# Guoxs/DODT

Measured on AMD Instinct MI355X. Metric: frame-pairs/sec (whole node) KITTI-shape tau=2, higher is better.
Workload: dtype f32

## Files before the change

dodt_amd/_lib.py:

```python
import ctypes as C
import os

_HERE = os.path.dirname(os.path.abspath(__file__))
LIB_PATH = os.environ.get('DODT_HIP_LIB') or os.path.join(_HERE, 'lib', 'libdodt_hip.so')

OK, ERR_INVALID, ERR_HIP, ERR_UNSUPPORTED = 0, 1, 2, 3
PTS_VELO_XYZI, PTS_CAM_3XN = 0, 1
EXTRACTOR_VGG_PYR = 0
EXTRACTOR_VGG = 1
EXTRACTOR_SHARED_GPU = 0x100
EXTRACTOR_BF16 = 0x200
EXTRACTOR_SPLIT = 0x400
FC_RELU = 1
FC_BF16 = 2
CONFLICT_RAISE, CONFLICT_NEXT_BEST = 0, 1


class DodtError(RuntimeError):
    pass


class BevParams(C.Structure):
    _fields_ = [
        ('point_format', C.c_int32),
        ('num_slices', C.c_int32),
        ('velo_to_cam', C.c_double * 12),
        ('p2', C.c_double * 12),
        ('im_w', C.c_double),
        ('im_h', C.c_double),
        ('plane', C.c_double * 4),
        ('extents', C.c_double * 6),
        ('voxel_size', C.c_double),
        ('height_lo', C.c_double),
        ('height_hi', C.c_double),
        ('occ_lo', C.c_double),
        ('occ_hi', C.c_double),
        ('has_pre_transform', C.c_int32),
        ('reserved_', C.c_int32),
        ('pre_translate', C.c_double * 3),
        ('pre_rotate', C.c_double * 9),
    ]


class LayerInfo(C.Structure):
    _fields_ = [('name', C.c_char * 32), ('kernel', C.c_char * 48), ('launches', C.c_int32),
                ('items', C.c_int32), ('flops_direct', C.c_double), ('flops_executed', C.c_double),
                ('bytes', C.c_double), ('ms', C.c_float), ('reserved_', C.c_int32)]


_vp = C.c_void_p
_i = C.c_int
_f = C.c_float
_d = C.c_double
_pi32 = C.c_void_p
_pf = C.c_void_p
_hf = C.c_void_p

SIGNATURES = {
    'dodt_version': (_i, []),
    'dodt_last_error': (C.c_char_p, []),
    'dodt_ctx_create': (_i, [_i, C.POINTER(_vp)]),
    'dodt_mark': (_i, [_vp, _i]),
    'dodt_ctx_wait_mark': (_i, [_vp, _vp, _i]),
    'dodt_mark_elapsed': (_i, [_vp, _i, _vp, _i, C.POINTER(_f)]),
    'dodt_ctx_create_high_priority': (_i, [_i, C.POINTER(_vp)]),
    'dodt_ctx_create_on_stream': (_i, [_i, _vp, C.POINTER(_vp)]),
    'dodt_ctx_destroy': (_i, [_vp]),
    'dodt_ctx_sync': (_i, [_vp]),
    'dodt_ctx_wait_for': (_i, [_vp, _vp]),
    'dodt_malloc': (_i, [_vp, C.c_size_t, C.POINTER(_vp)]),
    'dodt_free': (_i, [_vp, _vp]),
    'dodt_memcpy_h2d': (_i, [_vp, _vp, _vp, C.c_size_t]),
    'dodt_memcpy_d2h': (_i, [_vp, _vp, _vp, C.c_size_t]),
    'dodt_memset': (_i, [_vp, _vp, _i, C.c_size_t]),
    'dodt_pinned_alloc': (_i, [_vp, C.c_size_t, C.POINTER(_vp)]),
    'dodt_pinned_free': (_i, [_vp, _vp]),
    'dodt_memcpy_h2d_async': (_i, [_vp, _vp, _vp, C.c_size_t]),
    'dodt_fetch_i32_begin': (_i, [_vp, _pi32, _i, _i]),
    'dodt_fetch_i32_end': (_i, [_vp, _i, C.POINTER(C.c_int32), _i]),
    'dodt_timer_start': (_i, [_vp]),
    'dodt_timer_stop': (_i, [_vp, C.POINTER(_f)]),
    'dodt_bev_slices': (_i, [_vp, _vp, _i, C.POINTER(BevParams), _pf, _vp]),
    'dodt_bev_status': (_i, [_vp, C.POINTER(_i)]),
    'dodt_bev_support_mask': (_i, [C.POINTER(BevParams), _i, _vp, _i, _i]),
    'dodt_anchor_filter': (_i, [_vp, _vp, _i, _i, _pi32, _i, _i, _pi32, _pi32]),
    'dodt_project_anchors_f64': (_i, [_vp, _vp, _pi32, _i, _pi32,
                                      C.POINTER(_d), C.POINTER(_d), _d, _d,
                                      _pf, _pf, _pf]),
    'dodt_project_anchors_f32': (_i, [_vp, _pf, _i, _pi32, C.POINTER(_f),
                                      C.POINTER(_f), _f, _f, _pf, _pf, _pf]),
    'dodt_img_preprocess': (_i, [_vp, _vp, _i, _i, _i, _i, _i,
                                 C.POINTER(_f), _pf]),
    'dodt_conv_mode': (_i, []),
    'dodt_extractor_create': (_i, [_vp, _i, _i, _i, _i, _i, _i,
                                   C.POINTER(_vp)]),
    'dodt_extractor_destroy': (_i, [_vp]),
    'dodt_extractor_set_layer': (_i, [_vp, C.c_char_p, _vp, _i, _i, _i, _i,
                                      _vp, _vp, _vp]),
    'dodt_extractor_input': (_i, [_vp, C.POINTER(_vp), C.POINTER(C.c_longlong)]),
    'dodt_extractor_forward': (_i, [_vp, _pf, _pf, _pf]),
    'dodt_extractor_forward_padded': (_i, [_vp, _pf, _pf, _pf]),
    'dodt_extractor_set_input': (_i, [_vp, _pf]),
    'dodt_extractor_set_input_support': (_i, [_vp, _vp, _i, _i, C.POINTER(C.c_longlong)]),
    'dodt_extractor_set_frame_tables': (_i, [_vp, _i, C.POINTER(_i)]),
    'dodt_extractor_frame_items': (_i, [_vp, C.POINTER(_i), _i]),
    'dodt_extractor_frame_split': (_i, [_vp, C.POINTER(_i), C.POINTER(_i), _i]),
    'dodt_extractor_store_bytes': (C.c_longlong, [_vp]),
    'dodt_frame_tables_host': (_i, [_vp, _i, _i, _i, _i, _i, _i, _vp, _i, _vp, _vp, C.POINTER(_i)]),
    'dodt_frame_restore_host': (_i, [_vp, _i, _i, _i, _i, _i, _i, _i, _i, _i, _vp, _vp, _vp, _vp]),
    'dodt_frame_lists_host': (_i, [_vp, _i, _i, _i, _i, _i, _i, _vp, _i, _vp, _vp, C.POINTER(_i), _vp, C.POINTER(_i)]),
    'dodt_extractor_read_activation': (_i, [_vp, C.c_char_p, _vp,
                                            C.POINTER(_i), C.POINTER(_i),
                                            C.POINTER(_i)]),
    'dodt_extractor_output_shape': (_i, [_vp, C.POINTER(_i), C.POINTER(_i), C.POINTER(_i)]),
    'dodt_extractor_first_layers_folded': (_i, [_vp]),
    'dodt_extractor_flops': (_d, [_vp]),
    'dodt_extractor_mfma_flops': (_d, [_vp]),
    'dodt_extractor_bytes': (_d, [_vp]),
    'dodt_extractor_layer_count': (_i, [_vp]),
    'dodt_extractor_forward_timed': (_i, [_vp, _pf, _pf, _pf, C.POINTER(LayerInfo), _i]),
    'dodt_crop_and_resize': (_i, [_vp, _pf, _i, _i, _i, _pf, _i, _pi32, _i, _i,
                                  _pf]),
    'dodt_crop_and_resize_strided': (_i, [_vp, _pf, _i, _i, _i, _pf, _i, _pi32, _i, _i, _pf,
                                          C.c_longlong]),
    'dodt_correlation': (_i, [_vp, _pf, _pf, _i, _i, _i, _i, _i, _i, _pf]),
    'dodt_crop_and_resize_indexed': (_i, [_vp, _pf, _i, _i, _i, _pf, _i, _pi32, _i, _pi32, _i, _i, _pf,
                                          C.c_longlong]),
    'dodt_correlation_tile_list': (_i, [_vp, _i, _i, _pf, _i, _pi32, _i, _pi32, _i, _i, _pi32, _i, _pi32]),
    'dodt_correlation_tiles': (_i, [_vp, _pf, _pf, _i, _i, _i, _i, _i, _i, _pi32, _i, _pi32, _pf]),
    'dodt_mean_fusion': (_i, [_vp, _pf, _pf, _i, _pi32, _i, _pf]),
    'dodt_fc_create': (_i, [_vp, _i, _i, _hf, _hf, _i, C.POINTER(_vp)]),
    'dodt_fc_create_ex': (_i, [_vp, _i, _i, _hf, _hf, _i, C.POINTER(_vp)]),
    'dodt_fc_destroy': (_i, [_vp]),
    'dodt_fc_forward': (_i, [_vp, _vp, _pf, _pf, _i, _i, _pi32, _pf, _i]),
    'dodt_fc_forward_split': (_i, [_vp, _vp, _pf, _i, _i, _pi32, _i, C.POINTER(_i), C.POINTER(_vp)]),
    'dodt_fc_flops': (_d, [_vp, _i]),
    'dodt_fc_bf16_row_elems': (_i, [_vp]),
    'dodt_fc_forward_bf16': (_i, [_vp, _vp, _vp, _i, _i, _pi32, _vp, _i, _i]),
    'dodt_fc_forward_split_bf16': (_i, [_vp, _vp, _vp, _i, _i, _pi32, _i, C.POINTER(_i), C.POINTER(_vp)]),
    'dodt_rows_to_bf16': (_i, [_vp, _pf, _pf, _i, _pi32, _i, _i, _vp, _i]),
    'dodt_nms': (_i, [_vp, _pf, _pf, _i, _pi32, _i, _f, _pi32, _pi32]),
    'dodt_offset_to_anchor': (_i, [_vp, _pf, _pf, _i, _pi32, _pf]),
    'dodt_softmax_fg': (_i, [_vp, _pf, _i, _pi32, _pf]),
    'dodt_rpn_decode': (_i, [_vp, _pf, _pf, _pf, _i, _pi32, C.POINTER(_f), _pf, _pf, _pf]),
    'dodt_gather_project': (_i, [_vp, _pf, _pi32, _i, _pi32, C.POINTER(_f), C.POINTER(_f), _f, _f, _pf, _pf, _pf]),
    'dodt_final_decode': (_i, [_vp, _pf, _pf, _pf, _pf, _i, _pi32, C.POINTER(_f), C.POINTER(_f),
                               _pf, _pf, _pf, _pf, _pf, _pf]),
    'dodt_gather_rows': (_i, [_vp, _pf, _i, _pi32, _i, _pi32, _pf]),
    'dodt_max_fg_logit': (_i, [_vp, _pf, _i, _i, _pi32, _pf]),
    'dodt_pack_detections': (_i, [_vp, _pf, _pf, _pf, _pf, _pi32, _pi32, _i, _f, _pf, _pi32]),
    'dodt_pack_detections_compact': (_i, [_vp, _pf, _pf, _pf, _pf, _pi32, _pi32, _i, _f, _pf, _pi32]),
    'dodt_angle_vector_to_orientation': (_i, [_vp, _pf, _i, _pi32, _pf]),
    'dodt_class_scores': (_i, [_vp, _pf, _i, _i, _pi32, _pf, _pi32]),
    'dodt_final_decode_classes': (_i, [_vp, _pf, _pf, _pf, _i, _pf, _i, _pi32, C.POINTER(_f), C.POINTER(_f),
                                       _pf, _pf, _pf, _pf, _pf, _pi32, _pf]),
    'dodt_pack_detections_classes': (_i, [_vp, _pf, _pf, _pi32, _pf, _pf, _pi32, _pi32, _i, _f, _pf, _pi32]),
    'dodt_pack_detections_compact_classes': (_i, [_vp, _pf, _pf, _pi32, _pf, _pf, _pi32, _pi32, _i, _f, _pf, _pi32]),
    'dodt_box_4c_decode': (_i, [_vp, _pf, _pf, _i, _pi32, C.POINTER(_f),
                                C.POINTER(_f), _pf, _pf, _pf]),
    'dodt_comm_unique_id': (_i, [_vp]),
    'dodt_comm_create': (_i, [_vp, _i, _i, _vp, C.POINTER(_vp)]),
    'dodt_comm_destroy': (_i, [_vp]),
    'dodt_comm_attach': (_i, [_vp, _vp]),
    'dodt_comm_rank': (_i, [_vp, C.POINTER(_i), C.POINTER(_i)]),
    'dodt_comm_set_late_peer': (_i, [_vp, _d]),
    'dodt_all_gather_records': (_i, [_vp, _vp, _i, _pf, _pi32, _i, _i, _i, _i, _pf, _pi32]),
    'dodt_comm_join': (_i, [_vp, _i, _vp]),
    'dodt_comm_sync': (_i, [_vp]),
    'dodt_comm_barrier': (_i, [_vp]),
    'dodt_comm_max_f64': (_i, [_vp, C.POINTER(_d)]),
    'dodt_three_d_iou_matrix': (_i, [_vp, _vp, _i, _vp, _i, _vp]),
    'dodt_interpolate_pairs': (_i, [_vp, _vp, _i, _pi32, _i, _i, _i, _d, _i, _vp, C.POINTER(_d), _i, _vp,
                                    _pi32, _pi32]),
    'dodt_track_state_bytes': (_i, [_i, C.POINTER(C.c_size_t)]),
    'dodt_track_reset': (_i, [_vp, _vp, _i]),
    'dodt_track_flush': (_i, [_vp, _vp, _d, _i]),
    'dodt_track_encode': (_i, [_vp, _vp, _i, _pi32, _i, _i, C.POINTER(_d), _d, _d, _d, _pf, _pf, _pi32]),
    'dodt_track_pairs': (_i, [_vp, _vp, _vp, _i, _pi32, _i, _i, C.POINTER(_d), _d, _d, _d, _d, _d, _i]),
    'dodt_track_encoded': (_i, [_vp, _vp, _pf, _pf, _pi32, _i, _i, _d, _d, _i]),
}
COMM_ID_BYTES = 128

_lib = None


def load():
    global _lib
    if _lib is not None:
        return _lib
    if not os.path.exists(LIB_PATH):
        raise DodtError(
            'libdodt_hip.so not found at %s -- build it with '
            '`make -C dodt_amd/csrc` (there is no CPU fallback)' % LIB_PATH)
    lib = C.CDLL(LIB_PATH)
    for name, (res, args) in SIGNATURES.items():
        fn = getattr(lib, name)
        fn.restype = res
        fn.argtypes = args
    _lib = lib
    return lib


def check(rc, what=''):
    if rc == OK:
        return
    msg = load().dodt_last_error().decode('utf-8', 'replace')
    if rc == ERR_INVALID:
        raise ValueError(msg or what)
    raise DodtError('%s: %s (status %d)' % (what, msg, rc))
```

dodt_amd/core/models/anchor_predictor.py:

```python
import numpy as np

from dodt_amd import ops


class AnchorPredictor(object):
    def __init__(self, ctx, params, dtype='f32'):
        def mat(name):
            w = np.asarray(params[name]['w'], np.float32)
            return w.reshape(-1, w.shape[-1]), np.asarray(params[name]['b'], np.float32)
        wc, bc = mat('cls_fc6')
        wr, br = mat('reg_fc6')
        self.width = wc.shape[1]
        if wr.shape != wc.shape:
            raise ValueError('cls_fc6 and reg_fc6 must have the same size')
        self.fc6 = ops.FullyConnected(ctx, np.concatenate([wc, wr], 1),
                                      np.concatenate([bc, br]), True, dtype=dtype)
        self.cls7 = ops.FullyConnected(ctx, *mat('cls_fc7'), relu=True, dtype=dtype)
        self.reg7 = ops.FullyConnected(ctx, *mat('reg_fc7'), relu=True, dtype=dtype)
        self.cls8 = ops.FullyConnected(ctx, *mat('cls_fc8'), relu=False, dtype=dtype)
        self.reg8 = ops.FullyConnected(ctx, *mat('reg_fc8'), relu=False, dtype=dtype)
        self.layers = [self.fc6, self.cls7, self.reg7, self.cls8, self.reg8]
        (w8c, b8c), (w8r, b8r) = mat('cls_fc8'), mat('reg_fc8')
        w8 = np.zeros((w8c.shape[0] + w8r.shape[0], w8c.shape[1] + w8r.shape[1]), np.float32)
        w8[:w8c.shape[0], :w8c.shape[1]] = w8c
        w8[w8c.shape[0]:, w8c.shape[1]:] = w8r
        self.out8 = ops.FullyConnected(ctx, w8, np.concatenate([b8c, b8r]), False, dtype=dtype)
        if not (self.out8.can_split() and w8c.shape[0] == self.width == w8r.shape[0]):
            self.out8.close()
            self.out8 = None
        self.ctx = ctx

    def make_scratch(self, n_max):
        return [self.ctx.empty((n_max, 2 * self.width), np.float32) for _ in range(2)]

    def forward(self, ctx, d_bev_roi, d_img_roi, n, d_objectness, d_offsets, scratch):
        w = self.width
        h6, h7 = scratch
        self.fc6.forward(d_bev_roi, n, h6, d_x2=d_img_roi, ctx=ctx)
        self.cls7.forward(h6, n, h7, ldx=2 * w, ldy=2 * w, ctx=ctx)
        self.reg7.forward(h6.offset(4 * w, (1,)), n, h7.offset(4 * w, (1,)),
                          ldx=2 * w, ldy=2 * w, ctx=ctx)
        if self.out8 is not None:
            self.out8.forward_split(h7, n, [d_objectness, d_offsets], [self.cls8.N, self.reg8.N], ctx=ctx)
            return
        self.cls8.forward(h7, n, d_objectness, ldx=2 * w, ctx=ctx)
        self.reg8.forward(h7.offset(4 * w, (1,)), n, d_offsets, ldx=2 * w, ctx=ctx)

    def flops(self, n):
        return sum(l.flops(n) for l in self.layers)

    def close(self):
        for l in self.layers + ([self.out8] if self.out8 is not None else []):
            l.close()
```

dodt_amd/csrc/anchors.hip:

```cpp
#include "common.h"

namespace {

__device__ __forceinline__ int box_count(const uint32_t* __restrict__ occ, int wpr, int x1,
                                         int z1, int x2, int z2, int thr) {
    int cnt = 0;
    if (x2 <= x1) return 0;
    const int w0 = x1 >> 5, w1 = (x2 - 1) >> 5;
    for (int z = z1; z < z2; ++z) {
        for (int w = w0; w <= w1; ++w) {
            uint32_t word = occ[z * wpr + w];
            const int lo = (w == w0) ? (x1 & 31) : 0;
            const int hi = (w == w1) ? ((x2 - 1) & 31) : 31;
            uint32_t m = (hi == 31 ? 0xFFFFFFFFu : ((1u << (hi + 1)) - 1u)) & ~((1u << lo) - 1u);
            cnt += __popc(word & m);
        }
        if (cnt >= thr) return cnt;
    }
    return cnt;
}

constexpr int kMaskBlock = 64;
__global__ void __launch_bounds__(kMaskBlock)
anchor_mask_kernel(const uint32_t* __restrict__ occ, int wpr, int nx, int nz,
                   const int4* __restrict__ cells, int n, int thr,
                   uint8_t* __restrict__ mask, int* __restrict__ block_counts) {
    const int i = blockIdx.x * blockDim.x + threadIdx.x;
    int keep = 0;
    if (i < n) {
        int4 b = cells[i];
        const int x1 = min(max(b.x, 0), nx), z1 = min(max(b.y, 0), nz);
        const int x2 = min(max(b.z, 0), nx), z2 = min(max(b.w, 0), nz);
        keep = box_count(occ, wpr, x1, z1, x2, z2, thr) >= thr;
        mask[i] = (uint8_t)keep;
    }
    const int total = __popcll(__ballot(keep));
    if (threadIdx.x == 0) block_counts[blockIdx.x] = total;
}

__global__ void __launch_bounds__(256)
anchor_compact_kernel(const uint8_t* __restrict__ mask, const int* __restrict__ block_counts,
                      int n, int* __restrict__ keep_idx, int* __restrict__ count_out) {
    __shared__ int s_part[256];
    __shared__ int s_wave[4];
    const int tid = threadIdx.x;
    int part = 0;
    for (int j = tid; j < (int)blockIdx.x * (256 / kMaskBlock); j += 256) part += block_counts[j];
    s_part[tid] = part;
    __syncthreads();
    for (int s = 128; s > 0; s >>= 1) {
        if (tid < s) s_part[tid] += s_part[tid + s];
        __syncthreads();
    }
    const int block_off = s_part[0];
    const int i = blockIdx.x * 256 + tid;
    const int keep = (i < n) ? mask[i] : 0;
    const unsigned long long bal = __ballot(keep);
    const int lane = tid & 63, wave = tid >> 6;
    const int before = __popcll(bal & ((1ull << lane) - 1ull));
    if (lane == 0) s_wave[wave] = __popcll(bal);
    __syncthreads();
    int wave_off = 0;
    for (int w = 0; w < wave; ++w) wave_off += s_wave[w];
    if (keep) keep_idx[block_off + wave_off + before] = i;
    if (blockIdx.x == gridDim.x - 1 && tid == 0)
        *count_out = block_off + s_wave[0] + s_wave[1] + s_wave[2] + s_wave[3];
}

struct ProjParams64 {
    double x_min, x_max, z_min, z_max;
    double p[12];
    double im_w, im_h;
};

__device__ __forceinline__ void proj_corner64(const double* p, double x, double y, double z,
                                              double& u, double& v) {
    const double un = fma(p[2], z, fma(p[1], y, p[0] * x)) + p[3];
    const double vn = fma(p[6], z, fma(p[5], y, p[4] * x)) + p[7];
    const double w = fma(p[10], z, fma(p[9], y, p[8] * x)) + p[11];
    u = un / w;
    v = vn / w;
}

__global__ void __launch_bounds__(256)
project_f64_kernel(const double* __restrict__ anchors, const int* __restrict__ idx, int n,
                   const int* __restrict__ d_n, const ProjParams64 P,
                   float* __restrict__ bev_norm, float* __restrict__ img_norm,
                   float* __restrict__ anchors_f32) {
    const int i = blockIdx.x * blockDim.x + threadIdx.x;
    const int lim = d_n ? min(*d_n, n) : n;
    if (i >= lim) return;
    const int row = idx ? idx[i] : i;
    const double* a = anchors + (size_t)row * 6;
    const double x = a[0], y = a[1], z = a[2], dx = a[3], dy = a[4], dz = a[5];
    if (anchors_f32) {
        float* o = anchors_f32 + (size_t)i * 6;
        o[0] = (float)x; o[1] = (float)y; o[2] = (float)z;
        o[3] = (float)dx; o[4] = (float)dy; o[5] = (float)dz;
    }
    const double hx = dx / 2.0, hz = dz / 2.0;
    if (bev_norm) {
        const double xr = P.x_max - P.x_min, zr = P.z_max - P.z_min;
        const double x1 = (x - hx) - P.x_min, x2 = (x + hx) - P.x_min;
        const double z1 = (P.z_max - (z + hz)) - P.z_min, z2 = (P.z_max - (z - hz)) - P.z_min;
        float* o = bev_norm + (size_t)i * 4;
        o[0] = (float)(z1 / zr); o[1] = (float)(x1 / xr);
        o[2] = (float)(z2 / zr); o[3] = (float)(x2 / xr);
    }
    if (img_norm) {
        double umin = 1e300, umax = -1e300, vmin = 1e300, vmax = -1e300;
        const double xs[2] = {x + hx, x - hx};
        const double ys[2] = {y, y - dy};
        const double zs[2] = {z + hz, z - hz};
#pragma unroll
        for (int k = 0; k < 8; ++k) {
            double u, v;
            proj_corner64(P.p, xs[(k >> 1) & 1], ys[k >> 2], zs[((k + 1) >> 1) & 1], u, v);
            umin = (u < umin || u != u) ? u : umin; umax = (u > umax || u != u) ? u : umax;
            vmin = (v < vmin || v != v) ? v : vmin; vmax = (v > vmax || v != v) ? v : vmax;
        }
        float* o = img_norm + (size_t)i * 4;
        o[0] = (float)(vmin / P.im_h); o[1] = (float)(umin / P.im_w);
        o[2] = (float)(vmax / P.im_h); o[3] = (float)(umax / P.im_w);
    }
}

struct ProjParams32 {
    float x_min, x_max, z_min, z_max;
    float p[12];
    float im_w, im_h;
};

__device__ __forceinline__ void bev_box32(float x, float z, float dx, float dz,
                                          const ProjParams32& P, float& x1, float& z1,
                                          float& x2, float& z2) {
    const float hx = dx / 2.0f, hz = dz / 2.0f;
    x1 = (x - hx) - P.x_min;
    x2 = (x + hx) - P.x_min;
    z1 = (P.z_max - (z + hz)) - P.z_min;
    z2 = (P.z_max - (z - hz)) - P.z_min;
}

__device__ __forceinline__ void project_f32_elem(int i, float x, float y, float z, float dx, float dy, float dz,
                                                 const ProjParams32& P, float* __restrict__ bev,
                                                 float* __restrict__ bev_norm_tf, float* __restrict__ img_norm_tf) {
    float x1, z1, x2, z2;
    bev_box32(x, z, dx, dz, P, x1, z1, x2, z2);
    if (bev) {
        float* o = bev + (size_t)i * 4;
        o[0] = x1; o[1] = z1; o[2] = x2; o[3] = z2;
    }
    if (bev_norm_tf) {
        const float xr = P.x_max - P.x_min, zr = P.z_max - P.z_min;
        float* o = bev_norm_tf + (size_t)i * 4;
        o[0] = z1 / zr; o[1] = x1 / xr; o[2] = z2 / zr; o[3] = x2 / xr;
    }
    if (img_norm_tf) {
        const float hx = dx / 2.0f, hz = dz / 2.0f;
        const float xs[2] = {x + hx, x - hx};
        const float ys[2] = {y, y - dy};
        const float zs[2] = {z + hz, z - hz};
        float umin = 3.0e38f, umax = -3.0e38f, vmin = 3.0e38f, vmax = -3.0e38f;
#pragma unroll
        for (int k = 0; k < 8; ++k) {
            const float cx = xs[(k >> 1) & 1], cy = ys[k >> 2], cz = zs[((k + 1) >> 1) & 1];
            const float un = ((P.p[0] * cx + P.p[1] * cy) + P.p[2] * cz) + P.p[3];
            const float vn = ((P.p[4] * cx + P.p[5] * cy) + P.p[6] * cz) + P.p[7];
            const float w = ((P.p[8] * cx + P.p[9] * cy) + P.p[10] * cz) + P.p[11];
            const float u = un / w, v = vn / w;
            umin = fminf(umin, u); umax = fmaxf(umax, u);
            vmin = fminf(vmin, v); vmax = fmaxf(vmax, v);
        }
        float* o = img_norm_tf + (size_t)i * 4;
        o[0] = vmin / P.im_h; o[1] = umin / P.im_w; o[2] = vmax / P.im_h; o[3] = umax / P.im_w;
    }
}

__global__ void __launch_bounds__(256)
project_f32_kernel(const float* __restrict__ anchors, int n, const int* __restrict__ d_n,
                   const ProjParams32 P, float* __restrict__ bev, float* __restrict__ bev_norm_tf,
                   float* __restrict__ img_norm_tf) {
    const int i = blockIdx.x * blockDim.x + threadIdx.x;
    const int lim = d_n ? min(*d_n, n) : n;
    if (i >= lim) return;
    const float* a = anchors + (size_t)i * 6;
    project_f32_elem(i, a[0], a[1], a[2], a[3], a[4], a[5], P, bev, bev_norm_tf, img_norm_tf);
}

__device__ __forceinline__ void offset_to_anchor_elem(const float* __restrict__ a, const float* __restrict__ t, float o[6]) {
    o[0] = (t[0] * a[3]) + a[0];
    o[1] = (t[1] * a[4]) + a[1];
    o[2] = (t[2] * a[5]) + a[2];
    o[3] = expf(logf(a[3]) + t[3]);
    o[4] = expf(logf(a[4]) + t[4]);
    o[5] = expf(logf(a[5]) + t[5]);
}

__global__ void __launch_bounds__(256)
offset_to_anchor_kernel(const float* __restrict__ anchors, const float* __restrict__ off, int n,
                        const int* __restrict__ d_n, float* __restrict__ out) {
    const int i = blockIdx.x * blockDim.x + threadIdx.x;
    const int lim = d_n ? min(*d_n, n) : n;
    if (i >= lim) return;
    float o[6];
    offset_to_anchor_elem(anchors + (size_t)i * 6, off + (size_t)i * 6, o);
#pragma unroll
    for (int k = 0; k < 6; ++k) out[(size_t)i * 6 + k] = o[k];
}

__device__ __forceinline__ float softmax_fg_elem(float l0, float l1) {
    const float m = fmaxf(l0, l1);
    const float e0 = expf(l0 - m), e1 = expf(l1 - m);
    return e1 / (e0 + e1);
}

__global__ void __launch_bounds__(256)
softmax_fg_kernel(const float* __restrict__ logits, int n, const int* __restrict__ d_n,
                  float* __restrict__ out) {
    const int i = blockIdx.x * blockDim.x + threadIdx.x;
    const int lim = d_n ? min(*d_n, n) : n;
    if (i >= lim) return;
    out[i] = softmax_fg_elem(logits[2 * (size_t)i], logits[2 * (size_t)i + 1]);
}

__global__ void __launch_bounds__(256)
rpn_decode_kernel(const float* __restrict__ anchors, const float* __restrict__ off, const float* __restrict__ logits,
                  int n, const int* __restrict__ d_n, const ProjParams32 P, float* __restrict__ regressed,
                  float* __restrict__ bev_norm_tf, float* __restrict__ scores) {
    const int i = blockIdx.x * blockDim.x + threadIdx.x;
    const int lim = d_n ? min(*d_n, n) : n;
    if (i >= lim) return;
    float o[6];
    offset_to_anchor_elem(anchors + (size_t)i * 6, off + (size_t)i * 6, o);
#pragma unroll
    for (int k = 0; k < 6; ++k) regressed[(size_t)i * 6 + k] = o[k];
    project_f32_elem(i, o[0], o[1], o[2], o[3], o[4], o[5], P, nullptr, bev_norm_tf, nullptr);
    scores[i] = softmax_fg_elem(logits[2 * (size_t)i], logits[2 * (size_t)i + 1]);
}

__global__ void __launch_bounds__(256)
gather_project_kernel(const float* __restrict__ src, const int* __restrict__ idx, int n, const int* __restrict__ d_n,
                      const ProjParams32 P, float* __restrict__ rows, float* __restrict__ bev_norm_tf,
                      float* __restrict__ img_norm_tf) {
    const int i = blockIdx.x * blockDim.x + threadIdx.x;
    const int lim = d_n ? min(*d_n, n) : n;
    if (i >= lim) return;
    const float* a = src + (size_t)idx[i] * 6;
    float o[6];
#pragma unroll
    for (int k = 0; k < 6; ++k) { o[k] = a[k]; rows[(size_t)i * 6 + k] = o[k]; }
    project_f32_elem(i, o[0], o[1], o[2], o[3], o[4], o[5], P, nullptr, bev_norm_tf, img_norm_tf);
}

__global__ void __launch_bounds__(256)
gather_rows_kernel(const float* __restrict__ src, int width, const int* __restrict__ idx, int n,
                   const int* __restrict__ d_n, float* __restrict__ out) {
    const int t = blockIdx.x * blockDim.x + threadIdx.x;
    const int lim = d_n ? min(*d_n, n) : n;
    const int i = t / width, c = t - i * width;
    if (i >= lim) return;
    out[(size_t)i * width + c] = src[(size_t)idx[i] * width + c];
}

__global__ void __launch_bounds__(256)
max_fg_logit_kernel(const float* __restrict__ logits, int n_cls, int n,
                    const int* __restrict__ d_n, float* __restrict__ out) {
    const int i = blockIdx.x * blockDim.x + threadIdx.x;
    const int lim = d_n ? min(*d_n, n) : n;
    if (i >= lim) return;
    float m = logits[(size_t)i * n_cls + 1];
    for (int c = 2; c < n_cls; ++c) m = fmaxf(m, logits[(size_t)i * n_cls + c]);
    out[i] = m;
}

constexpr int kMaxClasses = 8;

__device__ __forceinline__ void class_scores_elem(const float* __restrict__ l, int n_cls, float& score, int& type,
                                                  float& nms) {
    float e[kMaxClasses];
    float m = l[0];
#pragma unroll
    for (int c = 1; c < kMaxClasses; ++c)
        if (c < n_cls) m = fmaxf(m, l[c]);
    float sum = 0.0f, fg = l[1];
#pragma unroll
    for (int c = 0; c < kMaxClasses; ++c)
        if (c < n_cls) {
            e[c] = expf(l[c] - m);
            sum = c ? sum + e[c] : e[c];
            if (c >= 2) fg = fmaxf(fg, l[c]);
        }
    float best = e[1] / sum;
    int arg = 0;
#pragma unroll
    for (int c = 2; c < kMaxClasses; ++c)
        if (c < n_cls) {
            const float p = e[c] / sum;
            if (p > best) { best = p; arg = c - 1; }
        }
    score = best;
    type = arg;
    nms = fg;
}

__global__ void __launch_bounds__(256)
class_scores_kernel(const float* __restrict__ logits, int n_cls, int n, const int* __restrict__ d_n,
                    float* __restrict__ scores, int* __restrict__ types) {
    const int i = blockIdx.x * blockDim.x + threadIdx.x;
    const int lim = d_n ? min(*d_n, n) : n;
    if (i >= lim) return;
    float score, nms;
    int type;
    class_scores_elem(logits + (size_t)i * n_cls, n_cls, score, type, nms);
    scores[i] = score;
    types[i] = type;
}

__device__ __forceinline__ void orientation_correct(float b[7], float ori) {
    const float kPi = (float)M_PI, kTwoPi = (float)(2.0 * M_PI);
    const float q1 = (float)(0.25 * M_PI), q2 = (float)(0.50 * M_PI), q3 = (float)(0.75 * M_PI);
    float diff = b[6] - ori;
    if (diff < -kPi) diff += kTwoPi;
    if (diff > kPi) diff -= kTwoPi;
    const bool pos = q1 < diff && diff < q3;
    const bool neg = -q1 > diff && diff > -q3;
    if (pos || neg) {
        const float l = b[3];
        b[3] = b[4];
        b[4] = l;
    }
    if (pos) b[6] += q2;
    if (neg) b[6] -= q2;
    if (fabsf(diff) >= q3) b[6] += kPi;
    if (b[6] > kPi) b[6] -= kTwoPi;
}

__global__ void __launch_bounds__(256)
pack_detections_kernel(const float* __restrict__ boxes_3d, const float* __restrict__ scores,
                       const float* __restrict__ orientations, const float* __restrict__ corr,
                       const int* __restrict__ sel, const int* __restrict__ d_count, int max_det,
                       float frame_mark, float* __restrict__ rec, int* __restrict__ count_out, int corr_compact,
                       const int* __restrict__ types) {
    const int t = blockIdx.x * blockDim.x + threadIdx.x;
    const int cnt = min(*d_count, max_det);
    if (t == 0) *count_out = cnt;
    if (t >= max_det * 17) return;
    const int row = t / 17, col = t - row * 17;
    float v = 0.0f;
    if (row < cnt) {
        const int src = sel[row];
        if (col == 7) v = scores[src];
        else if (col == 8) v = types ? (float)types[src] : 0.0f;
        else if (col == 16) v = frame_mark;
        else if (col < 7 || (col >= 9 && corr)) {
            float b[7];
#pragma unroll
            for (int k = 0; k < 7; ++k) b[k] = boxes_3d[(size_t)src * 7 + k];
            if (orientations) orientation_correct(b, orientations[src]);
            if (col >= 9) {
                const size_t cr = corr_compact ? row : src;
                b[0] += corr[cr * 3 + 0];
                b[2] += corr[cr * 3 + 1];
                b[6] += corr[cr * 3 + 2];
            }
            const int c = col < 7 ? col : col - 9;
#pragma unroll
            for (int k = 0; k < 7; ++k)
                if (k == c) v = b[k];
        }
    }
    rec[t] = v;
}

__global__ void __launch_bounds__(256)
angle_vector_to_orientation_kernel(const float* __restrict__ vec, int n,
                                   const int* __restrict__ d_n, float* __restrict__ out) {
    const int i = blockIdx.x * blockDim.x + threadIdx.x;
    if (d_n) n = min(n, *d_n);
    if (i < n) out[i] = atan2f(vec[2 * i + 1], vec[2 * i]);
}

__device__ __forceinline__ void box_info32(float vx, float vz, float mag, const float* px,
                                           const float* pz, float mx, float mz, float& cx,
                                           float& cz, float& len, float& wid, float& ry) {
    const float nx = vx / mag, nz = vz / mag;
    const float ox = -nz, oz = nx;
    float lmin = 3.0e38f, lmax = -3.0e38f, wmin = 3.0e38f, wmax = -3.0e38f;
#pragma unroll
    for (int k = 0; k < 4; ++k) {
        const float rx = px[k] - mx, rz = pz[k] - mz;
// ... 402 lines not shown
```

dodt_amd/csrc/crop.hip:

```cpp
#include "common.h"
#include "crop_coords.h"

namespace {

template <int VEC>
__global__ void __launch_bounds__(256)
crop_kernel(const float* __restrict__ img, int H, int W, int C, const float* __restrict__ boxes,
            int n, const int* __restrict__ d_n, int ch, int cw, float* __restrict__ out,
            long long out_stride, const int* __restrict__ box_idx, int n_boxes) {
    const int groups = C / VEC;
    const long long t = (long long)blockIdx.x * blockDim.x + threadIdx.x;
    const int lim = d_n ? min(*d_n, n) : n;
    const long long total = (long long)lim * ch * cw * groups;
    if (t >= total) return;
    const int g = (int)(t % groups);
    long long r = t / groups;
    const int ix = (int)(r % cw); r /= cw;
    const int iy = (int)(r % ch);
    const int b = (int)(r / ch);
    const int src = box_idx ? box_idx[b] : b;
    const bool have = !box_idx || (src >= 0 && src < n_boxes);
    const float4 bx = have ? reinterpret_cast<const float4*>(boxes)[src] : make_float4(0.f, 0.f, 0.f, 0.f);
    const float hm1 = (float)(H - 1), wm1 = (float)(W - 1);
    const float in_y = dodt::crop_coord(bx.x, bx.z, H, ch, iy);
    const float in_x = dodt::crop_coord(bx.y, bx.w, W, cw, ix);
    float* o = out + (size_t)b * out_stride + (((size_t)iy * cw + ix) * C + (size_t)g * VEC);
    const bool ok = have && (in_y >= 0.0f) && (in_y <= hm1) && (in_x >= 0.0f) && (in_x <= wm1);
    if (!ok) {
#pragma unroll
        for (int k = 0; k < VEC; ++k) o[k] = 0.0f;
        return;
    }
    const int ty = (int)floorf(in_y), by = (int)ceilf(in_y);
    const int lx_i = (int)floorf(in_x), rx_i = (int)ceilf(in_x);
    const float ly = in_y - (float)ty, lx = in_x - (float)lx_i;
    const float* ptl = img + ((size_t)ty * W + lx_i) * C + (size_t)g * VEC;
    const float* ptr = img + ((size_t)ty * W + rx_i) * C + (size_t)g * VEC;
    const float* pbl = img + ((size_t)by * W + lx_i) * C + (size_t)g * VEC;
    const float* pbr = img + ((size_t)by * W + rx_i) * C + (size_t)g * VEC;
#pragma unroll
    for (int k = 0; k < VEC; ++k) {
        const float tl = ptl[k], tr = ptr[k], bl = pbl[k], br = pbr[k];
        const float top = tl + (tr - tl) * lx;
        const float bot = bl + (br - bl) * lx;
        o[k] = top + (bot - top) * ly;
    }
}

int launch_crop(dodt_ctx* ctx, const float* d_image, int H, int W, int C, const float* d_boxes, int n,
                const int32_t* d_n, int crop_h, int crop_w, float* d_out, long long out_box_stride,
                const int32_t* d_box_idx, int n_boxes) {
    DODT_REQUIRE(ctx && d_image && d_out && (n == 0 || d_boxes),
                 "dodt_crop_and_resize: NULL argument");
    DODT_REQUIRE(H > 0 && W > 0 && C > 0 && crop_h > 0 && crop_w > 0 && n >= 0,
                 "dodt_crop_and_resize: bad sizes");
    DODT_REQUIRE(out_box_stride >= (long long)crop_h * crop_w * C,
                 "dodt_crop_and_resize: output stride %lld shorter than a crop", out_box_stride);
    if (n == 0) return DODT_OK;
    const int vec = (C % 4 == 0 && out_box_stride % 4 == 0) ? 4 : 1;
    const long long total = (long long)n * crop_h * crop_w * (C / vec);
    const int blocks = (int)((total + 255) / 256);
    if (vec == 4)
        hipLaunchKernelGGL(crop_kernel<4>, dim3(blocks), dim3(256), 0, ctx->stream, d_image, H, W,
                           C, d_boxes, n, d_n, crop_h, crop_w, d_out, out_box_stride, d_box_idx, n_boxes);
    else
        hipLaunchKernelGGL(crop_kernel<1>, dim3(blocks), dim3(256), 0, ctx->stream, d_image, H, W,
                           C, d_boxes, n, d_n, crop_h, crop_w, d_out, out_box_stride, d_box_idx, n_boxes);
    DODT_LAUNCH_CHECK();
    return DODT_OK;
}

}

extern "C" int dodt_crop_and_resize(dodt_ctx* ctx, const float* d_image, int H, int W, int C,
                                    const float* d_boxes, int n, const int32_t* d_n, int crop_h,
                                    int crop_w, float* d_out) {
    return dodt_crop_and_resize_strided(ctx, d_image, H, W, C, d_boxes, n, d_n, crop_h, crop_w, d_out,
                                        (long long)crop_h * crop_w * C);
}

extern "C" int dodt_crop_and_resize_strided(dodt_ctx* ctx, const float* d_image, int H, int W, int C,
                                            const float* d_boxes, int n, const int32_t* d_n, int crop_h,
                                            int crop_w, float* d_out, long long out_box_stride) {
    return launch_crop(ctx, d_image, H, W, C, d_boxes, n, d_n, crop_h, crop_w, d_out, out_box_stride, nullptr, n);
}

extern "C" int dodt_crop_and_resize_indexed(dodt_ctx* ctx, const float* d_image, int H, int W, int C,
                                            const float* d_boxes, int n_boxes, const int32_t* d_box_idx, int n,
                                            const int32_t* d_n, int crop_h, int crop_w, float* d_out,
                                            long long out_box_stride) {
    DODT_REQUIRE(d_box_idx && n_boxes >= 0, "dodt_crop_and_resize_indexed: NULL index list");
    return launch_crop(ctx, d_image, H, W, C, d_boxes, n, d_n, crop_h, crop_w, d_out, out_box_stride, d_box_idx,
                       n_boxes);
}
```

dodt_amd/csrc/crop_coords.h:

```cpp
#pragma once

namespace dodt {

__device__ __forceinline__ float crop_coord(float lo, float hi, int size, int crop, int i) {
    const float m1 = (float)(size - 1);
    const float step = (crop > 1) ? (hi - lo) * m1 / (float)(crop - 1) : 0.0f;
    return (crop > 1) ? lo * m1 + (float)i * step : 0.5f * (lo + hi) * m1;
}

}
```

dodt_amd/csrc/gemm.hip:

```cpp
#include <cmath>
#include <cstdlib>
#include <mutex>
#include <set>
#include <type_traits>
#include <vector>

#include <algorithm>

#include "common.h"
#include "lds_dma.h"

namespace {

typedef float f32x16 __attribute__((ext_vector_type(16)));
typedef float f32x4 __attribute__((ext_vector_type(4)));

constexpr int kKAlign = 64;
constexpr int kSmallK = 16;

struct GemmArgs {
    const float* x;
    const float* x2;
    const float* w;
    const float* bias;
    float* y;
    int M, K, Kp, N, ldx, ldy, relu;
    const int* d_m;
};

__device__ __forceinline__ int resolved_rows(const int* d_m, int M) { return d_m ? min(*d_m, M) : M; }

__device__ __forceinline__ int xcd_tile(int tiles) {
    int tile = blockIdx.x;
    if (tiles % 8 == 0) tile = (int)(blockIdx.x % 8) * (tiles / 8) + (int)(blockIdx.x / 8);
    return tile;
}

typedef __bf16 bf16x8 __attribute__((ext_vector_type(8)));
typedef __bf16 bf16x2 __attribute__((ext_vector_type(2)));
typedef float f32x2 __attribute__((ext_vector_type(2)));
__device__ __forceinline__ float pack_bf16(float lo, float hi) {
    return __builtin_bit_cast(float, __builtin_convertvector(f32x2{lo, hi}, bf16x2));
}

__device__ __forceinline__ float bf16_value(float packed, int which) {
    const unsigned u = __builtin_bit_cast(unsigned, packed);
    return __builtin_bit_cast(float, which ? (u & 0xffff0000u) : (u << 16));
}

template <bool YBF16>
__device__ __forceinline__ void store_tile32(const GemmArgs& a, const f32x16& acc, float b, int m_lane, int n, int M) {
#pragma unroll
    for (int r = 0; r < 16; ++r) {
        const int m = m_lane + (r & 3) + 8 * (r >> 2);
        if (m < M && n < a.N) {
            float v = acc[r] + b;
            if (a.relu) v = fmaxf(v, 0.0f);
            if constexpr (YBF16)
                reinterpret_cast<unsigned short*>(a.y)[(size_t)m * a.ldy + n] =
                    (unsigned short)(__builtin_bit_cast(unsigned, pack_bf16(v, 0.0f)) & 0xffffu);
            else
                a.y[(size_t)m * a.ldy + n] = v;
        }
    }
}

template <int BM, int BN, int WM, int WN, bool XVEC, int kBK, bool FUSE, bool BF16>
__global__ void __launch_bounds__(256)
fc_mfma_kernel(const GemmArgs a) {
    constexpr int MT = BM / 32 / WM, NT = BN / 32 / WN;
    constexpr int KB = BF16 ? 8 : 4;
    constexpr int G = kBK * 4 / KB;
    constexpr int kXS = G + 4;
    constexpr int XITEMS = BM * (G / 4);
    constexpr int WITEMS = G * BN / 4;
    constexpr int NX = (XITEMS + 255) / 256, NW = (WITEMS + 255) / 256;
    constexpr int kBuf = BM * kXS + G * BN;
    extern __shared__ __attribute__((aligned(16))) float smem[];

    const int tid = threadIdx.x, lane = tid & 63, wave = tid >> 6;
    const int wm = wave / WN, wn = wave % WN;
    const int li = lane & 31, lh = lane >> 5;
    const int m0 = blockIdx.x * BM, nt0 = blockIdx.y;
    const int M = resolved_rows(a.d_m, a.M);
    if (m0 >= M) return;
    const int nstages = a.Kp / kBK;
    const f32x4* wblk = reinterpret_cast<const f32x4*>(a.w) + (size_t)nt0 * (a.Kp / (2 * KB)) * 2 * BN;

    constexpr int XV = KB / 4;
    f32x4 prex[NX][XV];
    f32x4 pre[NX + NW];
    constexpr int NSLOT = NX + NW;
    int g_off[NSLOT];
    int l_off[NSLOT];
    int k_q[NX];
#pragma unroll
    for (int j = 0; j < NSLOT; ++j) {
        if (j < NX) {
            const int t = tid + j * 256;
            const int row = min(t / (G / 4), BM - 1), q = t % (G / 4);
            const int m = min(m0 + row, M - 1);
            g_off[j] = m * a.ldx + q * KB;
            k_q[j < NX ? j : 0] = q * KB;
            l_off[j] = row * kXS + q * 4;
        } else {
            const int t = min(tid + (j - NX) * 256, WITEMS - 1);
            g_off[j] = t;
            l_off[j] = BM * kXS + t * 4;
        }
    }
    f32x4 pre2[FUSE ? NX : 1][XV];
    auto load_slot = [&](int j, int st) {
        if (j < NX) {
            const int jx = j < NX ? j : 0;
            const int kk = st * kBK + k_q[jx];
            if constexpr (XVEC) {
                const int back = max(kk + KB - a.K, 0);
#pragma unroll
                for (int i = 0; i < XV; ++i) {
                    prex[jx][i] = *reinterpret_cast<const f32x4*>(a.x + g_off[j] + st * kBK +
                                                                  4 * i - back);
                    if constexpr (FUSE)
                        pre2[jx][i] = *reinterpret_cast<const f32x4*>(a.x2 + g_off[j] + st * kBK +
                                                                      4 * i - back);
                }
            } else {
#pragma unroll
                for (int e = 0; e < KB; ++e) {
                    const int back = max(kk + e + 1 - a.K, 0);
                    prex[jx][e / 4][e % 4] = a.x[g_off[j] + st * kBK + e - back];
                    if constexpr (FUSE)
                        pre2[jx][e / 4][e % 4] = a.x2[g_off[j] + st * kBK + e - back];
                }
            }
        } else {
            pre[j] = wblk[(size_t)st * (G / 4 * BN) + g_off[j]];
        }
    };
    auto store_slot = [&](int j, int buf, int st) {
        if (j < NX) {
            const int jx = j < NX ? j : 0;
            const int kk = st * kBK + k_q[jx];
            float v[KB];
#pragma unroll
            for (int e = 0; e < KB; ++e) {
                float t = prex[jx][e / 4][e % 4];
                if constexpr (FUSE) t = (t + pre2[jx][e / 4][e % 4]) / 2.0f;
                v[e] = (kk + e < a.K) ? t : 0.0f;
            }
            f32x4 o;
            if constexpr (BF16)
                o = f32x4{pack_bf16(v[0], v[1]), pack_bf16(v[2], v[3]),
                          pack_bf16(v[4 % KB], v[5 % KB]), pack_bf16(v[6 % KB], v[7 % KB])};
            else
                o = f32x4{v[0], v[1], v[2], v[3]};
            if (XITEMS % 256 == 0 || tid + j * 256 < XITEMS)
                *reinterpret_cast<f32x4*>(smem + buf * kBuf + l_off[j]) = o;
        } else {
            if (WITEMS % 256 == 0 || tid + (j - NX) * 256 < WITEMS)
                *reinterpret_cast<f32x4*>(smem + buf * kBuf + l_off[j]) = pre[j];
        }
    };
// ... 473 lines not shown
                    acc1 = mfma16x4(xv[u][s], wb[u][s], acc1);
                }
        }
    }
    s_part[wave][0][lane] = acc0;
    s_part[wave][1][lane] = acc1;
    __syncthreads();
    if (tid >= 128) return;
    const int nb = tid >> 6;
    f32x4 sum = s_part[0][nb][lane];
#pragma unroll
    for (int w = 1; w < 8; ++w) sum += s_part[w][nb][lane];
    const int n = nb * 16 + i;
    if (n >= a.N) return;
    const float b = a.bias[n];
    const int p = (n >= so.n_end[0]) + (n >= so.n_end[1]);
    float* y = p == 0 ? so.y[0] : (p == 1 ? so.y[1] : so.y[2]);
    const int ld = p == 0 ? so.ld[0] : (p == 1 ? so.ld[1] : so.ld[2]);
    const int nn = n - (p == 0 ? 0 : (p == 1 ? so.n_end[0] : so.n_end[1]));
#pragma unroll
    for (int r = 0; r < 4; ++r) {
        const int m = m0 + 4 * g + r;
        if (m < M) {
            float v = sum[r] + b;
            if (a.relu) v = fmaxf(v, 0.0f);
            y[(size_t)m * ld + nn] = v;
        }
    }
}

template <bool BF16>
__global__ void __launch_bounds__(256)
fc_smallk_kernel(const GemmArgs a, const float* __restrict__ w_plain) {
    const int M = resolved_rows(a.d_m, a.M);
    const int n4 = a.N >> 2;
    const long long t = (long long)blockIdx.x * blockDim.x + threadIdx.x;
    const int m = (int)(t / n4), c = (int)(t - (long long)m * n4) * 4;
    if (m >= M) return;
    const float* x = a.x + (size_t)m * a.ldx;
    const float* x2 = a.x2 ? a.x2 + (size_t)m * a.ldx : nullptr;
    f32x4 acc = {0.f, 0.f, 0.f, 0.f};
    for (int k = 0; k < a.K; ++k) {
        float xv = x[k];
        if (x2) xv = (xv + x2[k]) / 2.0f;
        if constexpr (BF16) xv = bf16_value(pack_bf16(xv, 0.0f), 0);
        const f32x4 wv = *reinterpret_cast<const f32x4*>(w_plain + (size_t)k * a.N + c);
        acc += wv * xv;
    }
    const f32x4 b = *reinterpret_cast<const f32x4*>(a.bias + c);
    acc += b;
    if (a.relu) {
#pragma unroll
        for (int i = 0; i < 4; ++i) acc[i] = fmaxf(acc[i], 0.0f);
    }
    float* y = a.y + (size_t)m * a.ldy + c;
    if ((a.ldy & 3) == 0) *reinterpret_cast<f32x4*>(y) = acc;
    else {
#pragma unroll
        for (int i = 0; i < 4; ++i) y[i] = acc[i];
    }
}

int launch_fc_skinny(hipStream_t s, const GemmArgs& a, const SplitOut& so, bool bf16, bool x_bf16) {
    if (x_bf16) hipLaunchKernelGGL((fc_skinny_kernel<true, true>), dim3(dodt::ceil_div(a.M, 16)), dim3(512), 0, s, a, so);
    else if (bf16) hipLaunchKernelGGL(fc_skinny_kernel<true>, dim3(dodt::ceil_div(a.M, 16)), dim3(512), 0, s, a, so);
    else hipLaunchKernelGGL(fc_skinny_kernel<false>, dim3(dodt::ceil_div(a.M, 16)), dim3(512), 0, s, a, so);
    DODT_LAUNCH_CHECK();
    return DODT_OK;
}

int launch_fc_smallk(hipStream_t s, const GemmArgs& a, const float* w_plain, bool bf16) {
    const long long threads = (long long)a.M * (a.N / 4);
    const dim3 grid((unsigned)((threads + 255) / 256));
    if (bf16) hipLaunchKernelGGL(fc_smallk_kernel<true>, grid, dim3(256), 0, s, a, w_plain);
    else hipLaunchKernelGGL(fc_smallk_kernel<false>, grid, dim3(256), 0, s, a, w_plain);
    DODT_LAUNCH_CHECK();
    return DODT_OK;
}

}

namespace {
__global__ void __launch_bounds__(256)
mean_fusion_kernel(const float4* __restrict__ a, const float4* __restrict__ b, int rows, const int* __restrict__ d_n,
                   int row4, float4* __restrict__ out) {
    const int lim = d_n ? min(*d_n, rows) : rows;
    const long long total = (long long)lim * row4;
    for (long long i = (long long)blockIdx.x * blockDim.x + threadIdx.x; i < total;
         i += (long long)gridDim.x * blockDim.x) {
        const float4 x = a[i], y = b[i];
        out[i] = make_float4((x.x + y.x) / 2.0f, (x.y + y.y) / 2.0f, (x.z + y.z) / 2.0f, (x.w + y.w) / 2.0f);
    }
}
}

extern "C" int dodt_mean_fusion(dodt_ctx* ctx, const float* d_a, const float* d_b, int rows, const int32_t* d_n,
                                int row_floats, float* d_out) {
    DODT_REQUIRE(ctx && d_a && d_b && d_out, "dodt_mean_fusion: NULL argument");
    DODT_REQUIRE(rows >= 0 && row_floats >= 4 && row_floats % 4 == 0,
                 "dodt_mean_fusion: rows of a multiple of four floats, got %d", row_floats);
    DODT_REQUIRE(((size_t)d_a | (size_t)d_b | (size_t)d_out) % 16 == 0, "dodt_mean_fusion: 16-byte aligned blocks");
    if (rows == 0) return DODT_OK;
    const long long total = (long long)rows * (row_floats / 4);
    const int blocks = (int)std::min<long long>((total + 255) / 256, 4096);
    hipLaunchKernelGGL(mean_fusion_kernel, dim3(blocks), dim3(256), 0, ctx->stream,
                       reinterpret_cast<const float4*>(d_a), reinterpret_cast<const float4*>(d_b), rows, d_n,
                       row_floats / 4, reinterpret_cast<float4*>(d_out));
    DODT_LAUNCH_CHECK();
    return DODT_OK;
}

namespace {
__global__ void __launch_bounds__(256)
rows_to_bf16_kernel(const float* __restrict__ a, const float* __restrict__ b, int rows, const int* __restrict__ d_n,
                    int row_floats, int in_ld, unsigned short* __restrict__ out, int out_ld) {
    const int lim = d_n ? min(*d_n, rows) : rows;
    const int q4 = out_ld / 4;
    const long long total = (long long)lim * q4;
    for (long long i = (long long)blockIdx.x * blockDim.x + threadIdx.x; i < total;
         i += (long long)gridDim.x * blockDim.x) {
        const int r = (int)(i / q4), c = (int)(i - (long long)r * q4) * 4;
        float v[4];
#pragma unroll
        for (int e = 0; e < 4; ++e) {
            float t = 0.0f;
            if (c + e < row_floats) {
                t = a[(size_t)r * in_ld + c + e];
                if (b) t = (t + b[(size_t)r * in_ld + c + e]) / 2.0f;
            }
            v[e] = t;
        }
        f32x2 o = {pack_bf16(v[0], v[1]), pack_bf16(v[2], v[3])};
        *reinterpret_cast<f32x2*>(out + (size_t)r * out_ld + c) = o;
    }
}
}

extern "C" int dodt_rows_to_bf16(dodt_ctx* ctx, const float* d_a, const float* d_b, int rows, const int32_t* d_n,
                                 int row_floats, int in_ld, void* d_out_bf16, int out_ld) {
    DODT_REQUIRE(ctx && d_a && d_out_bf16, "dodt_rows_to_bf16: NULL argument");
    DODT_REQUIRE(rows >= 0 && row_floats >= 1 && in_ld >= row_floats && out_ld >= row_floats && out_ld % 4 == 0,
                 "dodt_rows_to_bf16: rows of %d floats, %d apart, into rows of %d bf16 (a multiple of 4)", row_floats,
                 in_ld, out_ld);
    DODT_REQUIRE((size_t)d_out_bf16 % 8 == 0, "dodt_rows_to_bf16: 8-byte aligned output");
    if (rows == 0) return DODT_OK;
    const long long total = (long long)rows * (out_ld / 4);
    const int blocks = (int)std::min<long long>((total + 255) / 256, 4096);
    hipLaunchKernelGGL(rows_to_bf16_kernel, dim3(blocks), dim3(256), 0, ctx->stream, d_a, d_b, rows, d_n, row_floats,
                       in_ld, reinterpret_cast<unsigned short*>(d_out_bf16), out_ld);
    DODT_LAUNCH_CHECK();
    return DODT_OK;
}

struct dodt_fc {
    dodt_ctx* ctx = nullptr;
    int K = 0, Kp = 0, N = 0, Npad = 0, BN = 0, relu = 0;
    bool bf16 = false;
    float* d_w = nullptr;
    float* d_b = nullptr;
    float* d_w_plain = nullptr;
    void* d_w_dma = nullptr;
    int Kd = 0;
    int dma_bk = 0;
    bool smallk = false;
    bool skinny = false;
    bool dma = false;
};

namespace {

enum class FcForm {
    kNone,
    kSmallK,
    kSkinny,
    kSkinnyBf16,
    kSkinnyBf16Rows,
    kDmaNt1,
    kDmaNt2,
    kDmaFused,
    kBf16RowsDma32,
    kBf16RowsDma64,
    kTiled64x128,
    kTiled128x32,
    kTiled64x128Bf16,
    kTiled128x32Bf16,
};

FcForm select_fc_form(const dodt_fc& f, const GemmArgs& a, bool x_bf16, bool y_bf16) {
    if (x_bf16) {
        if (f.d_w_dma) return f.dma_bk == 64 ? FcForm::kBf16RowsDma64 : FcForm::kBf16RowsDma32;
        if (f.skinny && a.ldx % 4 == 0 && (size_t)a.x % 8 == 0 && !y_bf16) return FcForm::kSkinnyBf16Rows;
        return FcForm::kNone;
    }
    if (f.smallk && (size_t)a.y % 16 == 0) return FcForm::kSmallK;
    if (f.skinny && a.ldx % 4 == 0 && (size_t)a.x % 16 == 0 && !a.x2) return f.bf16 ? FcForm::kSkinnyBf16 : FcForm::kSkinny;
    if (f.bf16) {
        return f.BN == 128 ? FcForm::kTiled64x128Bf16 : FcForm::kTiled128x32Bf16;
    }
    if (f.BN != 128) return FcForm::kTiled128x32;
    if (f.dma && a.ldx % 4 == 0 && (size_t)a.x % 16 == 0 && (!a.x2 || (size_t)a.x2 % 16 == 0)) {
        if (a.x2) return FcForm::kDmaFused;
        const long tiles128 = (long)dodt::ceil_div(a.M, kDmaBM) * (f.Npad / 128);
        return tiles128 >= 2 * 256 ? FcForm::kDmaNt2 : FcForm::kDmaNt1;
    }
    return FcForm::kTiled64x128;
}

int launch_fc_form(FcForm form, const dodt_fc& f, hipStream_t s, GemmArgs a, const SplitOut& so, bool y_bf16) {
    switch (form) {
    case FcForm::kSmallK: return launch_fc_smallk(s, a, f.d_w_plain, f.bf16);
    case FcForm::kSkinny: return launch_fc_skinny(s, a, so, false, false);
    case FcForm::kSkinnyBf16: return launch_fc_skinny(s, a, so, true, false);
    case FcForm::kSkinnyBf16Rows: return launch_fc_skinny(s, a, so, true, true);
    case FcForm::kDmaNt1:
    case FcForm::kDmaFused: return launch_fc_dma(s, a, f.Npad, 1);
    case FcForm::kDmaNt2: return launch_fc_dma(s, a, f.Npad, 2);
    case FcForm::kBf16RowsDma32:
    case FcForm::kBf16RowsDma64:
        a.w = reinterpret_cast<const float*>(f.d_w_dma);
        a.Kp = f.Kd;
        return launch_fc_bf16_dma(s, a, f.Npad, y_bf16, f.dma_bk);
    case FcForm::kTiled64x128: return launch_fc<64, 128, 2, 2, 64, false>(s, a, f.Npad);
    case FcForm::kTiled128x32: return launch_fc<128, 32, 4, 1, 32, false>(s, a, f.Npad);
    case FcForm::kTiled64x128Bf16: return launch_fc<64, 128, 2, 2, 32, true>(s, a, f.Npad);
    case FcForm::kTiled128x32Bf16: return launch_fc<128, 32, 4, 1, 64, true>(s, a, f.Npad);
    case FcForm::kNone: break;
    }
    dodt::set_error("dodt_fc: no kernel form selected");
    return DODT_ERR_UNSUPPORTED;
}

GemmArgs fc_args(const dodt_fc& f, const void* d_x, const float* d_x2, int ldx, int M, const int32_t* d_m, void* d_y,
                 int ldy) {
    GemmArgs a;
    a.x = reinterpret_cast<const float*>(d_x); a.x2 = d_x2; a.w = f.d_w; a.bias = f.d_b; a.y = reinterpret_cast<float*>(d_y);
    a.M = M; a.K = f.K; a.Kp = f.Kp; a.N = f.N; a.ldx = ldx; a.ldy = ldy; a.relu = f.relu;
    a.d_m = d_m;
    return a;
}

SplitOut whole_out(const dodt_fc& f, void* d_y, int ldy) {
    float* y = reinterpret_cast<float*>(d_y);
    return SplitOut{{y, y, y}, {f.N, f.N, f.N}, {ldy, ldy, ldy}};
}

int split_out(const char* who, const dodt_fc& f, int parts, const int* widths, float* const* d_ys, SplitOut* so) {
    int end = 0;
    for (int p = 0; p < 3; ++p) {
        const int q = p < parts ? p : parts - 1;
        DODT_REQUIRE(widths[q] >= 1 && d_ys[q], "%s: part %d is empty", who, q);
        if (p < parts) end += widths[p];
        so->y[p] = d_ys[q];
        so->n_end[p] = p < parts ? end : f.N + 1;
        so->ld[p] = widths[q];
    }
    DODT_REQUIRE(end == f.N, "%s: the parts have %d columns, the layer %d", who, end, f.N);
    return DODT_OK;
}

}

extern "C" {

int dodt_fc_create(dodt_ctx* ctx, int K, int N, const float* w, const float* bias, int relu,
                   dodt_fc** out) {
    return dodt_fc_create_ex(ctx, K, N, w, bias, relu ? DODT_FC_RELU : 0, out);
}

int dodt_fc_create_ex(dodt_ctx* ctx, int K, int N, const float* w, const float* bias, int flags,
                      dodt_fc** out) {
    const int relu = (flags & DODT_FC_RELU) != 0;
    const bool bf16 = (flags & DODT_FC_BF16) != 0;
    DODT_REQUIRE(ctx && w && bias && out, "dodt_fc_create: NULL argument");
    DODT_REQUIRE(K >= 1 && N >= 1, "dodt_fc_create: bad sizes");
    dodt_fc* f = new dodt_fc();
    f->ctx = ctx;
    f->K = K;
    f->N = N;
    f->relu = relu;
    f->bf16 = bf16;
    f->Kp = (int)dodt::align_up((size_t)K, bf16 ? 2 * kKAlign : kKAlign);
    f->BN = (N >= 128) ? 128 : 32;
    f->Npad = (int)dodt::align_up((size_t)N, (size_t)f->BN);
    f->skinny = f->Npad == 32 && K % 16 == 0;
    f->dma = !bf16 && f->BN == 128 && K % kDmaBK == 0 && K >= 2 * kDmaBK;
    std::vector<float> blk((size_t)f->Kp * f->Npad, 0.0f), b(f->Npad, 0.0f);
    uint16_t* blk16 = reinterpret_cast<uint16_t*>(blk.data());
    const int kb = bf16 ? 8 : 4, KQ = f->Kp / (2 * kb);
    for (int k = 0; k < K; ++k)
        for (int n = 0; n < N; ++n) {
            const int q = k / (2 * kb), h = (k % (2 * kb)) / kb, s = k % kb;
            const int nt = n / f->BN, nn = n % f->BN;
            const size_t idx = ((((size_t)nt * KQ + q) * 2 + h) * f->BN + nn) * kb + s;
            if (bf16) blk16[idx] = dodt::float_to_bf16(w[(size_t)k * N + n]);
            else blk[idx] = w[(size_t)k * N + n];
        }
    for (int n = 0; n < N; ++n) b[n] = bias[n];
    hipError_t e1 = hipMalloc(&f->d_w, blk.size() * sizeof(float));
    hipError_t e2 = hipMalloc(&f->d_b, b.size() * sizeof(float));
    if (e1 != hipSuccess || e2 != hipSuccess) {
        dodt::set_error("dodt_fc_create: hipMalloc failed");
        dodt_fc_destroy(f);
        return DODT_ERR_HIP;
    }
    DODT_HIP_CHECK(hipMemcpyAsync(f->d_w, blk.data(), blk.size() * sizeof(float),
                                  hipMemcpyHostToDevice, ctx->stream));
    DODT_HIP_CHECK(hipMemcpyAsync(f->d_b, b.data(), b.size() * sizeof(float),
                                  hipMemcpyHostToDevice, ctx->stream));
    if (bf16 && N % kBfBN == 0 && K >= 128) {
        const int BK = bf16_dma_bk(), S = BK / 8;
        f->Kd = (int)dodt::align_up((size_t)K, (size_t)64);
        f->dma_bk = BK;
        const int ns = f->Kd / BK;
        std::vector<uint16_t> img((size_t)(N / kBfBN) * ns * kBfBN * BK, 0);
        for (int k = 0; k < K; ++k)
            for (int n = 0; n < N; ++n) {
                const int t = n / kBfBN, c = n % kBfBN, st = k / BK, kk = k % BK;
                const int slot = (kk / 8) ^ bf_swz(c, S);
                img[((((size_t)t * ns + st) * kBfBN + c) * S + slot) * 8 + kk % 8] = dodt::float_to_bf16(w[(size_t)k * N + n]);
            }
// ... 115 lines not shown
```

dodt_amd/ops.py:

```python
import ctypes as C

import numpy as np

from dodt_amd import _lib


def _arr(ctype, values):
    values = [float(v) for v in np.asarray(values, dtype=np.float64).reshape(-1)]
    return (ctype * len(values))(*values)


def _p(a):
    return None if a is None else C.c_void_p(a.ptr)


def make_bev_params(cfg, velo_to_cam=None, p2=None, im_wh=None,
                    point_format=_lib.PTS_VELO_XYZI, ground_plane=None,
                    area_extents=None, voxel_size=None):
    bp = _lib.BevParams()
    bp.point_format = point_format
    bp.num_slices = int(cfg['num_slices'])
    m = np.zeros(12) if velo_to_cam is None else \
        np.asarray(velo_to_cam, dtype=np.float64).reshape(-1)[:12]
    p = np.zeros(12) if p2 is None else np.asarray(p2, dtype=np.float64).reshape(-1)
# ... 15 lines not shown

def with_ego_motion(bev_params, trans, matrix):
    bp = _lib.BevParams.from_buffer_copy(bev_params)
    t = np.asarray(trans, np.float64).reshape(3)
    m = np.asarray(matrix, np.float64).reshape(9)
    bp.has_pre_transform = 1
    bp.pre_translate = (C.c_double * 3)(*t)
    bp.pre_rotate = (C.c_double * 9)(*m)
    return bp


def bev_slices(ctx, d_points, n_points, bev_params, d_bev_out, d_occ_bits=None):
    _lib.check(ctx.lib.dodt_bev_slices(ctx.handle, _p(d_points), int(n_points),
                                       C.byref(bev_params), _p(d_bev_out),
                                       _p(d_occ_bits)), 'dodt_bev_slices')


def bev_support_mask(bev_params, pad_top=0, lib=None):
    lib = lib or _lib.load()
    vs = bev_params.voxel_size
    ext = list(bev_params.extents)
    nx = int(np.ceil(ext[1] / vs - 1) - np.floor(ext[0] / vs) + 1)
    nz = int(np.ceil(ext[5] / vs - 1) - np.floor(ext[4] / vs) + 1)
    out = np.zeros((int(pad_top) + nz, nx), np.uint8)
    _lib.check(lib.dodt_bev_support_mask(C.byref(bev_params), int(pad_top), out.ctypes.data, out.shape[0],
                                         out.shape[1]), 'dodt_bev_support_mask')
    return out


def frame_tables_host(masks, layer, th, tw, items, prev=None, lib=None):
    lib = lib or _lib.load()
    masks = np.ascontiguousarray(masks, dtype=np.uint8)
    items = np.ascontiguousarray(items, dtype=np.int32).reshape(-1, 4)
    prev = None if prev is None else np.ascontiguousarray(prev, dtype=np.uint8)
    run = np.zeros((max(len(items), 1), 4), np.int32)
    n = C.c_int()
    _lib.check(lib.dodt_frame_tables_host(masks.ctypes.data, masks.shape[0], masks.shape[1], masks.shape[2], int(layer),
                                          int(th), int(tw), items.ctypes.data, len(items),
                                          None if prev is None else prev.ctypes.data, run.ctypes.data, C.byref(n)),
               'dodt_frame_tables_host')
    return run[:n.value].copy()


def frame_lists_host(masks, layer, th, tw, items, prev=None, lib=None):
    lib = lib or _lib.load()
    masks = np.ascontiguousarray(masks, dtype=np.uint8)
    items = np.ascontiguousarray(items, dtype=np.int32).reshape(-1, 4)
    prev = None if prev is None else np.ascontiguousarray(prev, dtype=np.uint8)
    run = np.zeros((max(len(items), 1), 4), np.int32)
    restore = np.zeros((max(len(items), 1), 4), np.int32)
    n, nr = C.c_int(), C.c_int()
    _lib.check(lib.dodt_frame_lists_host(masks.ctypes.data, masks.shape[0], masks.shape[1], masks.shape[2], int(layer),
                                         int(th), int(tw), items.ctypes.data, len(items),
                                         None if prev is None else prev.ctypes.data, run.ctypes.data, C.byref(n),
                                         restore.ctypes.data, C.byref(nr)),
               'dodt_frame_lists_host')
    return run[:n.value].copy(), restore[:nr.value].copy()


def frame_restore_host(item, f, th, tw, bn, ch0, dst, src, dst2=None, src2=None, pad_top=-1, lib=None):
    lib = lib or _lib.load()
    for a in (dst, src, dst2, src2):
        assert a is None or (a.dtype == np.float32 and a.flags.c_contiguous)
    item = np.ascontiguousarray(item, dtype=np.int32)
    if pad_top < 0:
        rows, cols, channels = dst.shape[2], dst.shape[3], dst.shape[1] * 8
    else:
        rows, cols, channels = dst.shape[1] + pad_top, dst.shape[2], dst.shape[3]
    _lib.check(lib.dodt_frame_restore_host(item.ctypes.data, int(f), int(th), int(tw), int(bn), int(ch0), rows, cols,
                                           channels, int(pad_top), dst.ctypes.data, src.ctypes.data,
                                           None if dst2 is None else dst2.ctypes.data,
                                           None if src2 is None else src2.ctypes.data), 'dodt_frame_restore_host')


def bev_status(ctx):
    f = C.c_int()
    _lib.check(ctx.lib.dodt_bev_status(ctx.handle, C.byref(f)), 'dodt_bev_status')
    return f.value


def anchor_filter(ctx, d_occ_bits, nx, nz, d_cells, n_anchors, d_keep_idx, d_count,
                  density_threshold=1):
    _lib.check(ctx.lib.dodt_anchor_filter(
        ctx.handle, _p(d_occ_bits), int(nx), int(nz), _p(d_cells), int(n_anchors),
        int(density_threshold), _p(d_keep_idx), _p(d_count)), 'dodt_anchor_filter')


def project_anchors_f64(ctx, d_anchors, d_idx, n, d_n, bev_extents, p2, im_wh,
                        d_bev_norm=None, d_img_norm=None, d_anchors_f32=None):
    _lib.check(ctx.lib.dodt_project_anchors_f64(
        ctx.handle, _p(d_anchors), _p(d_idx), int(n), _p(d_n),
        _arr(C.c_double, bev_extents), _arr(C.c_double, p2),
        float(im_wh[0]), float(im_wh[1]), _p(d_bev_norm), _p(d_img_norm),
        _p(d_anchors_f32)), 'dodt_project_anchors_f64')


def project_anchors_f32(ctx, d_anchors, n, d_n, bev_extents, p2, im_wh,
                        d_bev=None, d_bev_norm_tf=None, d_img_norm_tf=None):
    _lib.check(ctx.lib.dodt_project_anchors_f32(
        ctx.handle, _p(d_anchors), int(n), _p(d_n), _arr(C.c_float, bev_extents),
        _arr(C.c_float, p2), float(im_wh[0]), float(im_wh[1]), _p(d_bev),
        _p(d_bev_norm_tf), _p(d_img_norm_tf)), 'dodt_project_anchors_f32')


def img_preprocess(ctx, d_img_u8, in_hw, out_hw, out_c, mean_rgb, d_out):
    _lib.check(ctx.lib.dodt_img_preprocess(
        ctx.handle, _p(d_img_u8), int(in_hw[0]), int(in_hw[1]), int(out_hw[0]),
        int(out_hw[1]), int(out_c), _arr(C.c_float, mean_rgb), _p(d_out)),
        'dodt_img_preprocess')


def crop_and_resize(ctx, d_image, hwc, d_boxes, n, d_n, crop_hw, d_out, out_box_stride=None):
    if out_box_stride is None:
        out_box_stride = int(crop_hw[0]) * int(crop_hw[1]) * int(hwc[2])
    _lib.check(ctx.lib.dodt_crop_and_resize_strided(
        ctx.handle, _p(d_image), int(hwc[0]), int(hwc[1]), int(hwc[2]), _p(d_boxes),
        int(n), _p(d_n), int(crop_hw[0]), int(crop_hw[1]), _p(d_out), int(out_box_stride)),
        'dodt_crop_and_resize')


def crop_and_resize_indexed(ctx, d_image, hwc, d_boxes, n_boxes, d_box_idx, n, d_n, crop_hw, d_out,
                            out_box_stride=None):
    if out_box_stride is None:
        out_box_stride = int(crop_hw[0]) * int(crop_hw[1]) * int(hwc[2])
    _lib.check(ctx.lib.dodt_crop_and_resize_indexed(
        ctx.handle, _p(d_image), int(hwc[0]), int(hwc[1]), int(hwc[2]), _p(d_boxes), int(n_boxes),
        _p(d_box_idx), int(n), _p(d_n), int(crop_hw[0]), int(crop_hw[1]), _p(d_out), int(out_box_stride)),
        'dodt_crop_and_resize_indexed')


def nms(ctx, d_boxes, d_scores, n, d_n, max_out, iou_threshold, d_sel, d_count):
    _lib.check(ctx.lib.dodt_nms(
        ctx.handle, _p(d_boxes), _p(d_scores), int(n), _p(d_n), int(max_out),
        float(iou_threshold), _p(d_sel), _p(d_count)), 'dodt_nms')


def offset_to_anchor(ctx, d_anchors, d_offsets, n, d_n, d_out):
    _lib.check(ctx.lib.dodt_offset_to_anchor(
        ctx.handle, _p(d_anchors), _p(d_offsets), int(n), _p(d_n), _p(d_out)),
        'dodt_offset_to_anchor')


def softmax_fg(ctx, d_logits, n, d_n, d_scores):
    _lib.check(ctx.lib.dodt_softmax_fg(
        ctx.handle, _p(d_logits), int(n), _p(d_n), _p(d_scores)), 'dodt_softmax_fg')


def rpn_decode(ctx, d_anchors, d_offsets, d_logits, n, d_n, bev_extents, d_regressed, d_bev_norm_tf, d_scores):
    _lib.check(ctx.lib.dodt_rpn_decode(
        ctx.handle, _p(d_anchors), _p(d_offsets), _p(d_logits), int(n), _p(d_n), _arr(C.c_float, bev_extents),
        _p(d_regressed), _p(d_bev_norm_tf), _p(d_scores)), 'dodt_rpn_decode')


def gather_project(ctx, d_src, d_idx, n, d_n, bev_extents, p2, im_wh, d_rows, d_bev_norm_tf, d_img_norm_tf):
    _lib.check(ctx.lib.dodt_gather_project(
        ctx.handle, _p(d_src), _p(d_idx), int(n), _p(d_n), _arr(C.c_float, bev_extents), _arr(C.c_float, p2),
        float(im_wh[0]), float(im_wh[1]), _p(d_rows), _p(d_bev_norm_tf), _p(d_img_norm_tf)), 'dodt_gather_project')


def final_decode(ctx, d_top_anchors, d_offsets, d_cls_logits, d_angle_vectors, n, d_n, plane, bev_extents,
                 d_boxes_3d, d_pred_anchors, d_bev_tf, d_nms_scores, d_det_scores, d_orientations):
    _lib.check(ctx.lib.dodt_final_decode(
        ctx.handle, _p(d_top_anchors), _p(d_offsets), _p(d_cls_logits), _p(d_angle_vectors), int(n), _p(d_n),
        _arr(C.c_float, plane), _arr(C.c_float, bev_extents), _p(d_boxes_3d), _p(d_pred_anchors), _p(d_bev_tf),
        _p(d_nms_scores), _p(d_det_scores), _p(d_orientations)), 'dodt_final_decode')


def gather_rows(ctx, d_src, width, d_idx, n, d_n, d_out):
    _lib.check(ctx.lib.dodt_gather_rows(
        ctx.handle, _p(d_src), int(width), _p(d_idx), int(n), _p(d_n), _p(d_out)),
        'dodt_gather_rows')


def box_4c_decode(ctx, d_top_anchors, d_offsets, n, d_n, plane, bev_extents,
                  d_boxes_3d=None, d_pred_anchors=None, d_bev_tf=None):
    _lib.check(ctx.lib.dodt_box_4c_decode(
        ctx.handle, _p(d_top_anchors), _p(d_offsets), int(n), _p(d_n),
        _arr(C.c_float, plane), _arr(C.c_float, bev_extents), _p(d_boxes_3d),
        _p(d_pred_anchors), _p(d_bev_tf)), 'dodt_box_4c_decode')


def max_fg_logit(ctx, d_logits, n_cls, n, d_n, d_scores):
    _lib.check(ctx.lib.dodt_max_fg_logit(
        ctx.handle, _p(d_logits), int(n_cls), int(n), _p(d_n), _p(d_scores)),
        'dodt_max_fg_logit')


def angle_vector_to_orientation(ctx, d_angle_vectors, n, d_n, d_orientations):
    _lib.check(ctx.lib.dodt_angle_vector_to_orientation(
        ctx.handle, _p(d_angle_vectors), int(n), _p(d_n), _p(d_orientations)),
        'dodt_angle_vector_to_orientation')


def pack_detections(ctx, d_boxes_3d, d_scores, d_sel, d_count, max_det, frame_mark,
                    d_rec, d_count_out, d_corr_offsets=None, d_orientations=None):
    _lib.check(ctx.lib.dodt_pack_detections(
        ctx.handle, _p(d_boxes_3d), _p(d_scores), _p(d_orientations), _p(d_corr_offsets),
        _p(d_sel), _p(d_count), int(max_det), float(frame_mark), _p(d_rec), _p(d_count_out)),
        'dodt_pack_detections')


def pack_detections_compact(ctx, d_boxes_3d, d_scores, d_sel, d_count, max_det, frame_mark,
                            d_rec, d_count_out, d_det_offsets=None, d_orientations=None):
    _lib.check(ctx.lib.dodt_pack_detections_compact(
        ctx.handle, _p(d_boxes_3d), _p(d_scores), _p(d_orientations), _p(d_det_offsets),
        _p(d_sel), _p(d_count), int(max_det), float(frame_mark), _p(d_rec), _p(d_count_out)),
        'dodt_pack_detections_compact')


def class_scores(ctx, d_logits, n_cls, n, d_n, d_scores, d_types):
    _lib.check(ctx.lib.dodt_class_scores(
        ctx.handle, _p(d_logits), int(n_cls), int(n), _p(d_n), _p(d_scores), _p(d_types)), 'dodt_class_scores')


def final_decode_classes(ctx, d_top_anchors, d_offsets, d_cls_logits, n_cls, d_angle_vectors, n, d_n, plane,
                         bev_extents, d_boxes_3d, d_pred_anchors, d_bev_tf, d_nms_scores, d_det_scores, d_det_types,
                         d_orientations):
    _lib.check(ctx.lib.dodt_final_decode_classes(
        ctx.handle, _p(d_top_anchors), _p(d_offsets), _p(d_cls_logits), int(n_cls), _p(d_angle_vectors), int(n),
        _p(d_n), _arr(C.c_float, plane), _arr(C.c_float, bev_extents), _p(d_boxes_3d), _p(d_pred_anchors),
        _p(d_bev_tf), _p(d_nms_scores), _p(d_det_scores), _p(d_det_types), _p(d_orientations)),
        'dodt_final_decode_classes')


def pack_detections_classes(ctx, d_boxes_3d, d_scores, d_types, d_sel, d_count, max_det, frame_mark,
                            d_rec, d_count_out, d_corr_offsets=None, d_orientations=None):
    _lib.check(ctx.lib.dodt_pack_detections_classes(
        ctx.handle, _p(d_boxes_3d), _p(d_scores), _p(d_types), _p(d_orientations), _p(d_corr_offsets),
        _p(d_sel), _p(d_count), int(max_det), float(frame_mark), _p(d_rec), _p(d_count_out)),
        'dodt_pack_detections_classes')


def pack_detections_compact_classes(ctx, d_boxes_3d, d_scores, d_types, d_sel, d_count, max_det, frame_mark,
                                    d_rec, d_count_out, d_det_offsets=None, d_orientations=None):
    _lib.check(ctx.lib.dodt_pack_detections_compact_classes(
        ctx.handle, _p(d_boxes_3d), _p(d_scores), _p(d_types), _p(d_orientations), _p(d_det_offsets),
        _p(d_sel), _p(d_count), int(max_det), float(frame_mark), _p(d_rec), _p(d_count_out)),
        'dodt_pack_detections_compact_classes')


def fetch_i32_begin(ctx, d_src, n, slot):
    _lib.check(ctx.lib.dodt_fetch_i32_begin(ctx.handle, _p(d_src), int(n), int(slot)),
               'dodt_fetch_i32_begin')


def fetch_i32_end(ctx, slot, n):
    buf = (C.c_int32 * n)()
    _lib.check(ctx.lib.dodt_fetch_i32_end(ctx.handle, int(slot), buf, int(n)),
               'dodt_fetch_i32_end')
    return list(buf)


def correlation(ctx, d_a, d_b, hwc, max_displacement, stride_2, pad, d_out):
    _lib.check(ctx.lib.dodt_correlation(
        ctx.handle, _p(d_a), _p(d_b), int(hwc[0]), int(hwc[1]), int(hwc[2]),
        int(max_displacement), int(stride_2), int(pad), _p(d_out)), 'dodt_correlation')


def correlation_tile_list(ctx, out_hw, d_boxes, n_boxes, d_box_idx, n, d_n, crop_hw, d_tiles, capacity, d_n_tiles):
    _lib.check(ctx.lib.dodt_correlation_tile_list(
        ctx.handle, int(out_hw[0]), int(out_hw[1]), _p(d_boxes), int(n_boxes), _p(d_box_idx), int(n), _p(d_n),
        int(crop_hw[0]), int(crop_hw[1]), _p(d_tiles), int(capacity), _p(d_n_tiles)), 'dodt_correlation_tile_list')


def correlation_tiles(ctx, d_a, d_b, hwc, max_displacement, stride_2, pad, d_tiles, capacity, d_n_tiles, d_out):
    _lib.check(ctx.lib.dodt_correlation_tiles(
        ctx.handle, _p(d_a), _p(d_b), int(hwc[0]), int(hwc[1]), int(hwc[2]), int(max_displacement),
        int(stride_2), int(pad), _p(d_tiles), int(capacity), _p(d_n_tiles), _p(d_out)), 'dodt_correlation_tiles')


CORR_TILE_LIST_MAX = 8192


def correlation_tile_capacity(out_hw):
    return -(-int(out_hw[0]) // 16) * -(-int(out_hw[1]) // 16)


def mean_fusion(ctx, d_a, d_b, rows, d_n, row_floats, d_out):
    _lib.check(ctx.lib.dodt_mean_fusion(ctx.handle, _p(d_a), _p(d_b), int(rows), _p(d_n),
                                        int(row_floats), _p(d_out)), 'dodt_mean_fusion')


def rows_to_bf16(ctx, d_a, d_b, rows, d_n, row_floats, in_ld, d_out, out_ld):
    _lib.check(ctx.lib.dodt_rows_to_bf16(ctx.handle, _p(d_a), _p(d_b), int(rows), _p(d_n), int(row_floats),
                                         int(in_ld), _p(d_out), int(out_ld)), 'dodt_rows_to_bf16')


def bf16_to_float(a):
    return (np.asarray(a, np.uint16).astype(np.uint32) << 16).view(np.float32)


class FullyConnected(object):

    def __init__(self, ctx, w, b, relu, dtype='f32'):
        if dtype not in ('f32', 'bf16'):
            raise ValueError("dtype must be 'f32' or 'bf16'")
        w = np.ascontiguousarray(w, dtype=np.float32)
        b = np.ascontiguousarray(b, dtype=np.float32)
        if w.ndim != 2 or b.shape != (w.shape[1],):
            raise ValueError('weights must be (K,N) and bias (N,)')
        self.ctx, self.K, self.N, self.dtype = ctx, int(w.shape[0]), int(w.shape[1]), dtype
        h = C.c_void_p()
        flags = (_lib.FC_RELU if relu else 0) | (_lib.FC_BF16 if dtype == 'bf16' else 0)
        _lib.check(ctx.lib.dodt_fc_create_ex(ctx.handle, self.K, self.N,
                                             w.ctypes.data_as(C.c_void_p),
                                             b.ctypes.data_as(C.c_void_p), flags, C.byref(h)),
# ... 123 lines not shown
```

dodt_amd/pipeline.py:

```python
import os
from collections import namedtuple

import numpy as np

from dodt_amd import config as _config
from dodt_amd import _lib, device, ops, tracking
from dodt_amd.core.anchor_generators import grid_anchor_3d_generator as gen
from dodt_amd.core.avod_fc_layers.fusion_fc_layers import EarlyFusionFcLayers
from dodt_amd.core.feature_extractors.vgg import BevVgg, ImgVgg
from dodt_amd.core.feature_extractors.vgg_pyramid import BevVggPyr, ImgVggPyr
from dodt_amd.core.models.anchor_predictor import AnchorPredictor
from dodt_amd.temporal import unpack_frames

EXTRACTORS = {'vgg_pyr': (BevVggPyr, ImgVggPyr), 'vgg': (BevVgg, ImgVgg)}

MAX_DET = 100
REC_COLS = 17
ROI = 7
CORR_MAX_DISP, CORR_STRIDE2, CORR_PAD = 5, 2, 5
CORR_CH = (2 * (CORR_MAX_DISP // CORR_STRIDE2) + 1) ** 2

PREP_DONE_MARK = 244
TAIL_DONE_MARK = 247
CORR_MAP_MARK = 248
CONV_DONE_MARK = 250
PROPOSALS_MARK = 252
CORR_ROIS_MARK = 253


IMG_RING = 3
PREP_RING = 4
POINT_RING = 3

SeqSlots = namedtuple('SeqSlots', 'img prep points')


def sequence_slots(step, img_ring=IMG_RING, prep_ring=PREP_RING, point_ring=POINT_RING):
    return SeqSlots(img=(step % img_ring, (step + 1) % img_ring),
                    prep=(step % prep_ring, (step + 1) % prep_ring),
                    points=(step % point_ring, (step + 1) % point_ring))


class Schedule(namedtuple('Schedule', 'fused_tail no_tail no_corr no_rpn t_branch two_streams corr_map_img')):
    __slots__ = ()

    def t_placement(self, t_form):
        if not self.t_branch:
            return 'none', False
        if t_form == 'detections':
            return ('none' if self.no_corr else 'detections'), self.two_streams
        if self.no_corr:
            return 'none', False
        if not self.two_streams:
            return 'f0', False
        return ('img' if self.corr_map_img else 'f1'), False


def resolve_schedule(environ, computed_heads, frames_per_sample, n_side_streams):
    if environ is None:
        environ = os.environ
    return Schedule(fused_tail=environ.get('DODT_PIPE_FUSED_TAIL', '1') != '0',
                    no_tail=bool(environ.get('DODT_PIPE_NO_TAIL')), no_corr=bool(environ.get('DODT_PIPE_NO_CORR')),
                    no_rpn=bool(environ.get('DODT_PIPE_NO_RPN')),
                    t_branch=bool(computed_heads) and frames_per_sample == 2, two_streams=n_side_streams >= 2,
                    corr_map_img=environ.get('DODT_PIPE_CORR_MAP', 'img') == 'img')


_TailState = namedtuple('_TailState', 'step cur fr feat counts heads scratch')


class FramePairPipeline(object):

    def __init__(self, ctx, cfg, bev_params, img_params, p2=_config.KITTI_P2,
                 r0_rect=_config.KITTI_R0_RECT, tr_velo_to_cam=_config.KITTI_TR_VELO_TO_CAM,
                 image_wh=_config.KITTI_IMAGE_WH, n_points_max=120000, rpn_nms_size=1024,
                 pairs_per_step=1, side_streams=None, head_params=None, conv_dtype='f32',
                 head_dtype='f32', reuse_streams_of=None, temporal=None, tracker=None,
                 bev_input_skip=True, bev_frame_tables=True, t_branch_rows=None, sequence=False):
        self.sequence = bool(sequence)
        if self.sequence and (int(cfg.get('frames_per_sample', 2)) != 2 or int(pairs_per_step) != 1):
            raise ValueError('sequence: needs frames_per_sample == 2 and pairs_per_step == 1')
        if t_branch_rows not in (None, 'proposals', 'detections'):
            raise ValueError("t_branch_rows must be None, 'proposals' or 'detections'")
        self.t_branch_rows = t_branch_rows
        self._t_form = None
        self._caller_records = False
        self.ctx = ctx
        self.cfg = cfg
        self.p2 = np.asarray(p2, dtype=np.float64)
        self.image_wh = tuple(image_wh)
        self.P = int(rpn_nms_size)
        self.n_points_max = int(n_points_max)
        self.pairs = int(pairs_per_step)
        self.fps = int(cfg.get('frames_per_sample', 2))
        self.classes = tuple(cfg.get('classes', ('Car',)))
        self.n_cls = len(self.classes) + 1
        if not 2 <= self.n_cls <= 8:
            raise ValueError('1 to 7 classes')
        if self.fps not in (1, 2):
            raise ValueError('frames_per_sample must be 1 or 2')
        self.temporal = self._temporal_args(temporal)
        self.tracker = self._tracker_args(tracker)
        self.nf = self.fps * self.pairs
        self.bev_h, self.bev_w = cfg['bev_dims']
        self.img_h, self.img_w = cfg['img_dims']
        self.n_slices = cfg['num_slices']
        self.bev_extents_flat = np.asarray(cfg['bev_extents'], np.float64).reshape(-1)
        self.bp = ops.make_bev_params(cfg, _config.velo_to_cam(r0_rect, tr_velo_to_cam),
                                      self.p2, self.image_wh)
        if reuse_streams_of is not None:
            self.img_ctx, self.sides = reuse_streams_of.img_ctx, reuse_streams_of.sides
        else:
            self.img_ctx = device.Context(ctx.device_id)
            n_side = min(self.nf, 2) if side_streams is None else int(side_streams)
            self.sides = [device.Context(ctx.device_id) for _ in range(max(n_side, 1))]
        self.sched = resolve_schedule(None, head_params is not None, self.fps, len(self.sides))
        self.placement = self.alternate = None
        sizes, strides = _config.class_anchor_params(cfg)
        boxes = gen.tile_anchors_3d_classes(cfg['area_extents'], sizes, strides, cfg['ground_plane'])
        self.anchors_all = gen.box_3d_to_anchor(boxes)
        cells, self.nx, self.nz = gen.anchor_grid_cells(
            self.anchors_all, cfg['area_extents'], cfg['voxel_size'])
        self.n_all = len(self.anchors_all)
        self.d_anchor_table = ctx.array(self.anchors_all)
        self.d_cells = ctx.array(cells)

        bev_cls, img_cls = EXTRACTORS[cfg.get('extractor', 'vgg_pyr')]
        self.bev_net = bev_cls(ctx=ctx, shared_gpu=True, conv_dtype=conv_dtype)
        self.bev_net.load_params(bev_params)
        self.bev_net._ensure(self.nf, self.bev_h, self.bev_w, cfg['bev_depth'])
        self.bev_skipped_items = 0
        if bev_input_skip and conv_dtype == 'f32' and hasattr(self.bev_net, 'set_input_support') \
                and self.bp.point_format == _lib.PTS_VELO_XYZI:
            self.bev_skipped_items = self.bev_net.set_input_support(
                ops.bev_support_mask(self.bp, self.bev_net.PAD_TOP, ctx.lib), frame_tables=bev_frame_tables)
        self.img_net = img_cls(ctx=self.img_ctx, shared_gpu=True, conv_dtype=conv_dtype)
        self.img_net.load_params(img_params)
        n_img = 1 if self.sequence else self.nf
        self.img_net._ensure(n_img, self.img_h, self.img_w, 4)
        self.bev_fh, self.bev_fw, self.feat_c = self.bev_net.output_shape()
        self.img_fh, self.img_fw, img_c = self.img_net.output_shape()
        if img_c != self.feat_c:
            raise ValueError('mean fusion needs equal feature depths')
        self.bev_pad = self.bev_net.PAD_TOP
        self.in_bev = [ctx.zeros((self.nf, self.bev_pad + self.bev_h, self.bev_w, cfg['bev_depth']), np.float32)
                       for _ in range(2)]
        self.in_img = [ctx.zeros((n_img, self.img_net.PAD_TOP + self.img_h, self.img_w, 4), np.float32)
                       for _ in range(2)]
        self.bev_in = [self._views(a, (self.bev_h, self.bev_w, cfg['bev_depth']), self.bev_pad) for a in self.in_bev]
        self.img_in = [self._views(a, (self.img_h, self.img_w, 4), self.img_net.PAD_TOP, n_img) for a in self.in_img]
        self.d_bev_in = self.bev_in[0]

        f32, i32 = np.float32, np.int32
        N, P = self.n_all, self.P
        self.rpn_head = self.avod_head = self.corr_head = self.head_scratch = None
        rep = cfg.get('box_representation', 'box_4ca')
        if rep not in ('box_4c', 'box_4ca'):
            raise NotImplementedError('Regression not implemented for %s' % rep)
        self.box_4ca = rep == 'box_4ca'
        if head_params is not None:
            self.rpn_head = AnchorPredictor(ctx, head_params['rpn'], dtype=head_dtype)
            self.avod_head = EarlyFusionFcLayers(
                ctx, head_params['avod'], dtype=head_dtype,
                outputs=('cls_out', 'off_out') + (('ang_out',) if self.box_4ca else ()))
            if self.fps == 2:
                self.corr_head = EarlyFusionFcLayers(ctx, head_params['corr'],
                                                     outputs=('off_out',), dtype=head_dtype)
            self.head_scratch = [dict(rpn=self.rpn_head.make_scratch(N), fc=self.avod_head.make_scratch(P),
                                      corr_map=ctx.empty((self.bev_fh, self.bev_fw, CORR_CH), f32)
                                      if self.fps == 2 else None) for _ in self.sides]
            self.corr_maps = None
            if t_branch_rows == 'detections' and self.corr_head is not None and not self._tile_list_fits():
                raise ValueError("t_branch_rows='detections': the %d x %d map has more than %d tiles"
                                 % (self.bev_fh, self.bev_fw, ops.CORR_TILE_LIST_MAX))

        FC = self.feat_c
        self.feat = []
        for _ in range(2):
            d = dict(bev_feat=ctx.empty((self.nf, self.bev_fh, self.bev_fw, FC), f32),
                     bev_bneck=ctx.empty((self.nf, self.bev_fh, self.bev_fw, 1), f32))
            if not self.sequence:
                d.update(img_feat=ctx.empty((self.nf, self.img_fh, self.img_fw, FC), f32),
                         img_bneck=ctx.empty((self.nf, self.img_fh, self.img_fw, 1), f32))
            self.feat.append(d)
        if self.sequence:
            self.img_ring = [dict(img_feat=ctx.empty((1, self.img_fh, self.img_fw, FC), f32),
                                  img_bneck=ctx.empty((1, self.img_fh, self.img_fw, 1), f32)) for _ in range(IMG_RING)]
        self.feat_views = [[{name: a.offset(a.nbytes // self.nf * f, a.shape[1:]) for name, a in d.items()}
                            for f in range(self.nf)] for d in self.feat]
        def prep_set():
            return dict(occ=ctx.empty((self.nz, (self.nx + 31) // 32), np.uint32),
                        keep=ctx.empty((N,), i32), count=ctx.zeros((1,), i32),
                        bev_norm=ctx.empty((N, 4), f32), img_norm=ctx.empty((N, 4), f32),
                        anchors=ctx.empty((N, 6), f32))
        if self.sequence:
            self.prep_sets = [prep_set() for _ in range(PREP_RING)]
            self.seq_counts = [None] * PREP_RING
            self.pts_ring = [ctx.empty((self.n_points_max, 4), f32) for _ in range(POINT_RING)]
            self.pts_n = [0] * POINT_RING
            self.d_row_ids = ctx.array(np.arange(self.n_points_max, dtype=i32))
            self.seq_primed = False
            self.seq_prime_parity = None
        else:
            self.prep3 = [[prep_set() for _ in range(self.nf)] for _ in range(3)]
        if 3 * self.nf > 32:
            raise ValueError('at most 10 frames per step (count fetch slots)')
        self.fr2 = [[], []]
        for f in range(2 * self.nf):
            b = dict(
                rpn_bev_roi=ctx.empty((N, 3, 3, 1), f32), rpn_img_roi=ctx.empty((N, 3, 3, 1), f32),
                regressed=ctx.empty((N, 6), f32), prop_bev=ctx.empty((N, 4), f32),
                scores=ctx.empty((N,), f32),
                top_idx=ctx.empty((P,), i32), top_count=ctx.zeros((1,), i32),
                top_anchors=ctx.empty((P, 6), f32),
                top_bev=ctx.empty((P, 4), f32), top_img=ctx.empty((P, 4), f32),
                bev_rois=ctx.empty((P, ROI, ROI, FC), f32),
                img_rois=ctx.empty((P, ROI, ROI, FC), f32),
                boxes_3d=ctx.empty((P, 7), f32), pred_anchors=ctx.empty((P, 6), f32),
                nms2_boxes=ctx.empty((P, 4), f32), nms2_scores=ctx.empty((P,), f32),
                det_idx=ctx.empty((MAX_DET,), i32), det_count=ctx.zeros((1,), i32),
                det_scores=ctx.empty((P,), f32), orientations=ctx.empty((P,), f32))
            if self.n_cls > 2:
                b.update(det_types=ctx.zeros((P,), i32))
            if head_params is not None:
                b.update(rpn_logits=ctx.empty((N, 2), f32), rpn_offsets=ctx.empty((N, 6), f32),
                         cls_logits=ctx.empty((P, self.n_cls), f32), offsets_4c=ctx.empty((P, 10), f32))
                if self.box_4ca:
                    b.update(angle_vectors=ctx.empty((P, 2), f32))
                if self.fps == 2 and f % 2 == 0:
                    b.update(corr_rois=ctx.zeros((P, self.corr_head.in_ld), f32),
                             corr_offsets=ctx.empty((P, 3), f32))
            self.fr2[f // self.nf].append(b)
        self.fr = [dict(b, **p) for b, p in zip(self.fr2[0], self.prep_sets if self.sequence else self.prep3[0])]
        self.prepped = -1
        self.step_idx = 0
        self.pending = None
        self.rec2 = [ctx.empty((self.pairs, self.fps, MAX_DET, REC_COLS), f32) for _ in range(2)]
        self.cnt2 = [ctx.zeros((self.pairs, self.fps), i32) for _ in range(2)]
        self.d_records, self.d_rec_counts = self.rec2[0], self.cnt2[0]
        self.last_anchor_counts = [0] * self.nf
        self.on_records_reuse = None
        if self.temporal is not None:
            self.temporal_calib = ops.temporal_calib(r0_rect, tr_velo_to_cam)
            self._alloc_frames()
        if self.tracker is not None:
            tk = self.tracker
            self.track_state = tracking.Tracker(self.ctx, tk['max_sequence_dets'], tk['high_threshold'],
                                                tk['iou_threshold'], tk['t_min'], tk['score_threshold'])
            self.img_ctx.wait_for(self.ctx)
            self.last_sequence_tracks = None
        self.mark_steps = ()
        self.marks = {}
        ctx.sync()

    def _temporal_args(self, temporal):
        if temporal is None:
            return None
        if self.fps != 2:
            raise ValueError('temporal: needs frame pairs (frames_per_sample == 2)')
        t = dict(temporal)
        tm = dict(n_frames=int(t.pop('n_frames')), threshold=float(t.pop('threshold', 0.1)),
                  on_conflict=t.pop('on_conflict', 'raise'))
        if t:
            raise ValueError('temporal: unknown keys %s' % sorted(t))
        if tm['on_conflict'] not in ('raise', 'next_best'):
            raise ValueError("temporal: on_conflict must be 'raise' or 'next_best'")
        if not 1 <= tm['n_frames'] <= 64:
            raise ValueError('temporal: n_frames must be 1..64')
        return tm

    def _tracker_args(self, tracker):
        if tracker is None:
            return None
        if self.fps != 2:
            raise ValueError('tracker: needs frame pairs (frames_per_sample == 2)')
        t = dict(tracker)
        tk = dict(score_threshold=float(t.pop('score_threshold', 0.1)),
                  high_threshold=float(t.pop('high_threshold', 0.5)),
                  iou_threshold=float(t.pop('iou_threshold', 0.005)), t_min=int(t.pop('t_min', 3)),
                  classes=tuple(t.pop('classes', self.classes)), max_sequence_dets=int(t.pop('max_sequence_dets', 65536)))
        if t:
            raise ValueError('tracker: unknown keys %s' % sorted(t))
        if tk['max_sequence_dets'] < 1:
            raise ValueError('tracker: max_sequence_dets must be >= 1')
        return tk

    def _mark(self, c, step, name):
        if step in self.mark_steps:
            slot = sum(1 for (cc, _) in self.marks.values() if cc is c)
            if slot < 64:
                c.mark(slot)
                self.marks['%d:%s' % (step, name)] = (c, slot)

    def _views(self, arr, shape, pad_top=0, n=None):
        row = int(np.prod(shape[1:])) * 4
        frame = (pad_top + shape[0]) * row
        return [arr.offset(frame * f + pad_top * row, shape) for f in range(self.nf if n is None else n)]

    def _tile_list_fits(self):
        return ops.correlation_tile_capacity((self.bev_fh, self.bev_fw)) <= ops.CORR_TILE_LIST_MAX

    def t_branch_form(self):
        if self._t_form is not None:
            return self._t_form
        if self.t_branch_rows is not None:
            return self.t_branch_rows
        return 'detections' if self._caller_records and self._tile_list_fits() else 'proposals'

    def _t_detections(self):
        return self.corr_head is not None and self.t_branch_form() == 'detections'

    def _resolve_t_branch(self):
        if self._t_form is not None:
            return
        self._t_form = self.t_branch_form()
        self.placement, self.alternate = self.sched.t_placement(self._t_form)
        if self.corr_head is None:
            return
        ctx, f32, i32 = self.ctx, np.float32, np.int32
        if self._t_form == 'proposals':
# ... 298 lines not shown
            self._temporal_step(st)
            self._tracker_step(st)
            self.ctx.wait_for(self.img_ctx)

    def _temporal_step(self, st):
        if self.temporal is None:
            return
        T, r, c = self.temporal, st['rslot'], self.img_ctx
        self._mark(c, st['step'], 'temporal_start')
        ops.interpolate_pairs(c, self.rec2[r], self.cnt2[r], self.pairs, MAX_DET, T['n_frames'], T['threshold'],
                              T['on_conflict'], self.frames2[r], self.fcnt2[r], self.fst2[r],
                              d_recover=self.ego2[r] if st['recover'] else None,
                              calib=self.temporal_calib if st['recover'] else None, max_out=2 * MAX_DET)
        self._mark(c, st['step'], 'temporal_end')
        self.d_frames, self.d_frame_counts, self.d_frame_status = self.frames2[r], self.fcnt2[r], self.fst2[r]

    def _tracker_step(self, st):
        if self.tracker is None:
            return
        r, c = st['rslot'], self.img_ctx
        self._mark(c, st['step'], 'tracker_start')
        self.track_state.track_records(self.rec2[r], self.cnt2[r], self.pairs, MAX_DET, self.p2, self.image_wh, ctx=c)
        self._mark(c, st['step'], 'tracker_end')

    def _frame_ids(self, frame_ids):
        if frame_ids is not None:
            ids = [tuple(f) for f in frame_ids]
            return lambda pair, kf: ids[pair][kf]
        tau = self.temporal['n_frames'] - 1 if self.temporal is not None else 1
        return lambda pair, kf: pair * tau + kf * tau

    def tracks_so_far(self, frame_ids=None):
        if self.tracker is None:
            raise ValueError('tracks_so_far: the pipeline has no tracker')
        self.ctx.wait_for(self.img_ctx)
        return tracking.tracks_from_log(self.track_state.read(), self._frame_ids(frame_ids), self.tracker['classes'])

    def end_sequence(self, frame_ids=None):
        if self.tracker is None and not self.sequence:
            raise ValueError('end_sequence: the pipeline has no tracker')
        if self.pending is not None:
            raise ValueError('end_sequence: call finish() first (the last step is not tracked yet)')
        if self.sequence:
            self.seq_primed, self.prepped = False, -1
            if self.tracker is None:
                return None
        self.track_state.flush(ctx=self.img_ctx)
        tracks = self.tracks_so_far(frame_ids)
        self.track_state.reset(ctx=self.img_ctx)
        self.last_sequence_tracks = tracks
        return tracks

    def kitti_tracking_rows(self, tracks=None):
        from dodt_amd.core.dt_evaluator_utils import convert_trajectory_to_kitti_format
        if tracks is None:
            if self.tracker is None or self.last_sequence_tracks is None:
                raise ValueError('kitti_tracking_rows: no sequence has ended')
            tracks = self.last_sequence_tracks
        return convert_trajectory_to_kitti_format(tracks)

    def frames(self):
        if self.temporal is None:
            raise ValueError('frames: the pipeline has no temporal module')
        self.ctx.wait_for(self.img_ctx)
        return unpack_frames(self.d_frames.download(), self.d_frame_counts.download(),
                             self.d_frame_status.download(), self.temporal['on_conflict'])

    def _wait_convs(self, st):
        for s in self.sides:
            s.wait_mark(self.ctx, CONV_DONE_MARK + st['cur'])
            s.wait_mark(self.img_ctx, CONV_DONE_MARK + st['cur'])

    def _tail(self, st):
        cur, k3, nf, ns = st['cur'], st['step'] % 3, self.nf, len(self.sides)
        if self.sequence:
            counts, preps, feat = self._seq_tail_inputs(st)
        else:
            counts = [ops.fetch_i32_end(self.sides[f % ns], 3 * f + k3, 1)[0] for f in range(nf)]
            preps, feat = self.prep3[k3], self.feat_views[cur]
        self.last_anchor_counts = counts
        self.fr = [dict(b, **p) for b, p in zip(self.fr2[cur], preps)]
        self.d_records, self.d_rec_counts = self.rec2[st['rslot']], self.cnt2[st['rslot']]
        self.d_bev_in = self.bev_in[cur]
        if self.sched.no_tail:
            return
        if self.on_records_reuse is not None:
            self.on_records_reuse(st['rslot'], self.sides)
        t = _TailState(step=st['step'], cur=cur, fr=self.fr, feat=feat, counts=counts,
                       heads=self.fr if st['heads'] is None else st['heads'], scratch=self.head_scratch)
        if self.placement == 'img':
            for f0 in range(0, nf, 2):
                self._pair_img(t, f0)
        elif self.placement == 'f1':
            for f0 in range(0, nf, 2):
                self._pair_f1(t, f0)
        elif self.alternate:
            for f0 in range(0, nf, 2):
                for stage in (self._proposals, self._head2, self._decode_nms2, self._records):
                    stage(t, f0)
                    stage(t, f0 + 1)
        else:
            for f in range(nf):
                self._proposals(t, f)
                self._head2(t, f)
                if self.placement == 'f0' and f % 2 == 0:
                    self._t_map_crops(t, f, on=f)
                    self._mark(self.sides[f % ns], t.step, 'tail%d_corrmap' % f)
                    self._t_head(t, f, on=f)
                self._decode_nms2(t, f)
                self._records(t, f)

    def _pair_img(self, t, f0):
        ns = len(self.sides)
        c0, c1 = self.sides[f0 % ns], self.sides[(f0 + 1) % ns]
        self._proposals(t, f0)
        c0.mark(PROPOSALS_MARK)
        self._head2(t, f0)
        self._decode_nms2(t, f0)
        self._proposals(t, f0 + 1)
        c1.wait_mark(c0, PROPOSALS_MARK)
        c1.wait_mark(self.img_ctx, CORR_MAP_MARK + t.cur)
        self._t_crops(t, f0, f0 + 1, self.corr_maps[t.cur][f0 // 2])
        self._t_head(t, f0, on=f0 + 1)
        c1.mark(CORR_ROIS_MARK)
        c0.wait_mark(c1, CORR_ROIS_MARK)
        self._records(t, f0)
        self._head2(t, f0 + 1)
        self._decode_nms2(t, f0 + 1)
        self._records(t, f0 + 1)

    def _pair_f1(self, t, f0):
        ns = len(self.sides)
        c0, c1 = self.sides[f0 % ns], self.sides[(f0 + 1) % ns]
        self._proposals(t, f0)
        c0.mark(PROPOSALS_MARK)
        self._head2(t, f0)
        self._proposals(t, f0 + 1)
        c1.wait_mark(c0, PROPOSALS_MARK)
        self._t_map_crops(t, f0, on=f0 + 1)
        c1.mark(CORR_ROIS_MARK)
        self._head2(t, f0 + 1)
        self._decode_nms2(t, f0 + 1)
        self._records(t, f0 + 1)
        c0.wait_mark(c1, CORR_ROIS_MARK)
        self._mark(c0, t.step, 'tail%d_corrmap' % f0)
        self._t_head(t, f0, on=f0)
        self._decode_nms2(t, f0)
        self._records(t, f0)

    def _proposals(self, t, f):
        c, b, h, A, v = self.sides[f % len(self.sides)], t.fr[f], t.heads[f], t.counts[f], t.feat[f]
        bev_hw, img_hw, FC = (self.bev_fh, self.bev_fw), (self.img_fh, self.img_fw), self.feat_c
        self._mark(c, t.step, 'tail%d_start' % f)
        ops.crop_and_resize(c, v['bev_bneck'], bev_hw + (1,), b['bev_norm'], A, None, (3, 3), b['rpn_bev_roi'])
        ops.crop_and_resize(c, v['img_bneck'], img_hw + (1,), b['img_norm'], A, None, (3, 3), b['rpn_img_roi'])
        self._mark(c, t.step, 'tail%d_crops' % f)
        if self.rpn_head is not None and not self.sched.no_rpn:
            self.rpn_head.forward(c, b['rpn_bev_roi'], b['rpn_img_roi'], A, b['rpn_logits'],
                                  b['rpn_offsets'], t.scratch[f % len(self.sides)]['rpn'])
        self._mark(c, t.step, 'tail%d_rpn' % f)
        if self.sched.fused_tail:
            ops.rpn_decode(c, b['anchors'], h['rpn_offsets'], h['rpn_logits'], A, None, self.bev_extents_flat,
                           b['regressed'], b['prop_bev'], b['scores'])
        else:
            ops.offset_to_anchor(c, b['anchors'], h['rpn_offsets'], A, None, b['regressed'])
            ops.project_anchors_f32(c, b['regressed'], A, None, self.bev_extents_flat, self.p2,
                                    self.image_wh, d_bev_norm_tf=b['prop_bev'])
            ops.softmax_fg(c, h['rpn_logits'], A, None, b['scores'])
        ops.nms(c, b['prop_bev'], b['scores'], A, None, self.P, self.cfg['rpn_nms_iou_thresh'], b['top_idx'], b['top_count'])
        if self.sched.fused_tail:
            ops.gather_project(c, b['regressed'], b['top_idx'], self.P, b['top_count'], self.bev_extents_flat,
                               self.p2, self.image_wh, b['top_anchors'], b['top_bev'], b['top_img'])
            self._mark(c, t.step, 'tail%d_nms1' % f)
        else:
            ops.gather_rows(c, b['regressed'], 6, b['top_idx'], self.P, b['top_count'], b['top_anchors'])
            self._mark(c, t.step, 'tail%d_nms1' % f)
            ops.project_anchors_f32(c, b['top_anchors'], self.P, b['top_count'], self.bev_extents_flat, self.p2,
                                    self.image_wh, d_bev_norm_tf=b['top_bev'], d_img_norm_tf=b['top_img'])
        ops.crop_and_resize(c, v['bev_feat'], bev_hw + (FC,), b['top_bev'], self.P, b['top_count'], (ROI, ROI),
                            b['bev_rois'])
        ops.crop_and_resize(c, v['img_feat'], img_hw + (FC,), b['top_img'], self.P, b['top_count'], (ROI, ROI),
                            b['img_rois'])

    def _head2(self, t, f):
        c, b = self.sides[f % len(self.sides)], t.fr[f]
        self._mark(c, t.step, 'tail%d_crops2' % f)
        if self.rpn_head is not None:
            self.avod_head.forward(c, b['bev_rois'], b['img_rois'], self.P, b['top_count'],
                                   [b['cls_logits'], b['offsets_4c']] + ([b['angle_vectors']] if self.box_4ca else []),
                                   t.scratch[f % len(self.sides)]['fc'])
            self._mark(c, t.step, 'tail%d_fc2' % f)

    def _correlation_map(self, c, cur, f0, d_map):
        v = self.feat_views[cur]
        ops.correlation(c, v[f0]['bev_feat'], v[f0 + 1]['bev_feat'], (self.bev_fh, self.bev_fw, self.feat_c),
                        CORR_MAX_DISP, CORR_STRIDE2, CORR_PAD, d_map)

    def _t_crops(self, t, f0, on, d_map):
        b = t.fr[f0]
        ops.crop_and_resize(self.sides[on % len(self.sides)], d_map, (self.bev_fh, self.bev_fw, CORR_CH), b['top_bev'],
                            self.P, b['top_count'], (ROI, ROI), b['corr_rois'], out_box_stride=self.corr_head.in_ld)

    def _t_map_crops(self, t, f0, on):
        i = on % len(self.sides)
        self._correlation_map(self.sides[i], t.cur, f0, t.scratch[i]['corr_map'])
        self._t_crops(t, f0, on, t.scratch[i]['corr_map'])

    def _t_head(self, t, f0, on):
        i, b = on % len(self.sides), t.fr[f0]
        self.corr_head.forward(self.sides[i], b['corr_rois'], None, self.P, b['top_count'], [b['corr_offsets']],
                               t.scratch[i]['fc'])

    def _decode_nms2(self, t, f):
        c, b, h, plane = self.sides[f % len(self.sides)], t.fr[f], t.heads[f], self.cfg['ground_plane']
        self._mark(c, t.step, 'tail%d_heads' % f)
        if self.n_cls > 2:
            return self._decode_nms2_classes(c, b, h, plane)
        if self.sched.fused_tail:
            ops.final_decode(c, b['top_anchors'], h['offsets_4c'], h['cls_logits'],
                             h['angle_vectors'] if self.box_4ca else None, self.P, b['top_count'], plane,
                             self.bev_extents_flat, b['boxes_3d'], b['pred_anchors'], b['nms2_boxes'],
                             b['nms2_scores'], b['det_scores'], b['orientations'] if self.box_4ca else None)
            ops.nms(c, b['nms2_boxes'], b['nms2_scores'], self.P, b['top_count'], MAX_DET,
                    self.cfg['avod_nms_iou_thresh'], b['det_idx'], b['det_count'])
        else:
            ops.box_4c_decode(c, b['top_anchors'], h['offsets_4c'], self.P, b['top_count'],
                              plane, self.bev_extents_flat, b['boxes_3d'], b['pred_anchors'], b['nms2_boxes'])
            ops.max_fg_logit(c, h['cls_logits'], 2, self.P, b['top_count'], b['nms2_scores'])
            ops.nms(c, b['nms2_boxes'], b['nms2_scores'], self.P, b['top_count'], MAX_DET,
                    self.cfg['avod_nms_iou_thresh'], b['det_idx'], b['det_count'])
            ops.softmax_fg(c, h['cls_logits'], self.P, b['top_count'], b['det_scores'])
            if self.box_4ca:
                ops.angle_vector_to_orientation(c, h['angle_vectors'], self.P, b['top_count'], b['orientations'])

    def _decode_nms2_classes(self, c, b, h, plane):
        if self.sched.fused_tail:
            ops.final_decode_classes(c, b['top_anchors'], h['offsets_4c'], h['cls_logits'], self.n_cls,
                                     h['angle_vectors'] if self.box_4ca else None, self.P, b['top_count'], plane,
                                     self.bev_extents_flat, b['boxes_3d'], b['pred_anchors'], b['nms2_boxes'],
                                     b['nms2_scores'], b['det_scores'], b['det_types'],
                                     b['orientations'] if self.box_4ca else None)
            ops.nms(c, b['nms2_boxes'], b['nms2_scores'], self.P, b['top_count'], MAX_DET,
                    self.cfg['avod_nms_iou_thresh'], b['det_idx'], b['det_count'])
        else:
            ops.box_4c_decode(c, b['top_anchors'], h['offsets_4c'], self.P, b['top_count'],
                              plane, self.bev_extents_flat, b['boxes_3d'], b['pred_anchors'], b['nms2_boxes'])
            ops.max_fg_logit(c, h['cls_logits'], self.n_cls, self.P, b['top_count'], b['nms2_scores'])
            ops.nms(c, b['nms2_boxes'], b['nms2_scores'], self.P, b['top_count'], MAX_DET,
                    self.cfg['avod_nms_iou_thresh'], b['det_idx'], b['det_count'])
            ops.class_scores(c, h['cls_logits'], self.n_cls, self.P, b['top_count'], b['det_scores'], b['det_types'])
            if self.box_4ca:
                ops.angle_vector_to_orientation(c, h['angle_vectors'], self.P, b['top_count'], b['orientations'])

    def _records(self, t, f):
        c, b = self.sides[f % len(self.sides)], t.fr[f]
        frame0 = self.fps == 2 and f % 2 == 0
        d_rec = self.d_records.offset(4 * MAX_DET * REC_COLS * f, (MAX_DET, REC_COLS))
        d_cnt = self.d_rec_counts.offset(4 * f, (1,), np.int32)
        d_orient = b['orientations'] if self.box_4ca else None
        if self.n_cls > 2:
            types, pack, pack_compact = (b['det_types'],), ops.pack_detections_classes, ops.pack_detections_compact_classes
        else:
            types, pack, pack_compact = (), ops.pack_detections, ops.pack_detections_compact
        if frame0 and self._t_detections():
            if self.placement == 'detections':
                self._t_detection_rows(t, f)
            pack_compact(c, b['boxes_3d'], b['det_scores'], *types, b['det_idx'], b['det_count'], MAX_DET,
                         float(f % self.fps), d_rec, d_cnt, d_det_offsets=b['det_corr_offsets'], d_orientations=d_orient)
        else:
            pack(c, b['boxes_3d'], b['det_scores'], *types, b['det_idx'], b['det_count'], MAX_DET,
                 float(f % self.fps), d_rec, d_cnt,
                 d_corr_offsets=t.heads[f].get('corr_offsets') if frame0 else None, d_orientations=d_orient)
        self._mark(c, t.step, 'tail%d_end' % f)

    def _t_detection_rows(self, t, f):
        i = f % len(self.sides)
        c, b, scratch, v = self.sides[i], t.fr[f], t.scratch[i], t.feat
        bev_hw, FC = (self.bev_fh, self.bev_fw), self.feat_c
        ops.correlation_tile_list(c, bev_hw, b['top_bev'], self.P, b['det_idx'], MAX_DET, b['det_count'],
                                  (ROI, ROI), scratch['corr_tiles'], self.corr_tile_cap, scratch['corr_ntiles'])
        ops.correlation_tiles(c, v[f]['bev_feat'], v[f + 1]['bev_feat'], bev_hw + (FC,), CORR_MAX_DISP, CORR_STRIDE2,
                              CORR_PAD, scratch['corr_tiles'], self.corr_tile_cap, scratch['corr_ntiles'],
                              scratch['corr_map'])
        self._mark(c, t.step, 'tail%d_corrmap' % f)
        ops.crop_and_resize_indexed(c, scratch['corr_map'], bev_hw + (CORR_CH,), b['top_bev'], self.P,
                                    b['det_idx'], MAX_DET, b['det_count'], (ROI, ROI),
                                    b['det_corr_rois'], out_box_stride=self.corr_head.in_ld)
        self.corr_head.forward(c, b['det_corr_rois'], None, MAX_DET, b['det_count'],
                               [b['det_corr_offsets']], scratch['fc'])

    def sync(self):
        self.ctx.sync()

    def flops_per_step(self):
        return self.bev_net.flops() + self.img_net.flops()

    def mfma_flops_per_step(self):
        return self.bev_net.mfma_flops() + self.img_net.mfma_flops()

    def conv_bytes_per_step(self):
        return self.bev_net.bytes() + self.img_net.bytes()

    def head_flops_per_step(self, anchor_counts=None):
        if self.rpn_head is None:
            return 0.0
        counts = anchor_counts or self.last_anchor_counts
        return (sum(self.rpn_head.flops(a) for a in counts)
                + self.nf * self.avod_head.flops(self.P)
                + (self.pairs * self.corr_head.flops(MAX_DET if self._t_detections() else self.P)
                   if self.corr_head else 0.0))

    def flops_per_pair(self):
        return self.flops_per_step() / self.pairs

    def close(self):
        self.bev_net.close()
        self.img_net.close()
        for hd in (self.rpn_head, self.avod_head, self.corr_head):
            if hd is not None:
                hd.close()
```

include/dodt_hip.h:

```cpp
#ifndef DODT_HIP_H
#define DODT_HIP_H

#include <stddef.h>
#include <stdint.h>

#ifdef __cplusplus
extern "C" {
#endif

#define DODT_OK 0
#define DODT_ERR_INVALID 1
#define DODT_ERR_HIP 2
#define DODT_ERR_UNSUPPORTED 3

typedef struct dodt_ctx dodt_ctx;

int dodt_version(void);
const char* dodt_last_error(void);
int dodt_ctx_create(int device_id, dodt_ctx** out);
int dodt_ctx_create_high_priority(int device_id, dodt_ctx** out);
int dodt_ctx_create_on_stream(int device_id, void* hip_stream, dodt_ctx** out);
int dodt_ctx_destroy(dodt_ctx* ctx);
int dodt_ctx_sync(dodt_ctx* ctx);
int dodt_mark(dodt_ctx* ctx, int slot);
// ... 21 lines not shown
typedef struct dodt_bev_params {
    int32_t point_format;
    int32_t num_slices;
    double velo_to_cam[12];
    double p2[12];
    double im_w, im_h;
    double plane[4];
    double extents[6];
    double voxel_size;
    double height_lo, height_hi;
    double occ_lo, occ_hi;
    int32_t has_pre_transform;
    int32_t reserved_;
    double pre_translate[3];
    double pre_rotate[9];
} dodt_bev_params;

int dodt_bev_slices(dodt_ctx* ctx, const void* d_points, int n_points,
                    const dodt_bev_params* params, float* d_bev_out,
                    uint32_t* d_occ_bits_out);
int dodt_bev_status(dodt_ctx* ctx, int* flags);
int dodt_bev_support_mask(const dodt_bev_params* params, int pad_top, uint8_t* mask_out, int rows, int cols);

int dodt_anchor_filter(dodt_ctx* ctx, const uint32_t* d_occ_bits, int nx, int nz,
                       const int32_t* d_anchor_cells, int n_anchors,
                       int density_threshold, int32_t* d_keep_idx_out,
                       int32_t* d_count_out);

int dodt_project_anchors_f64(dodt_ctx* ctx, const double* d_anchors,
                             const int32_t* d_idx, int n, const int32_t* d_n,
                             const double bev_extents[4], const double p2[12],
                             double im_w, double im_h, float* d_bev_norm_out,
                             float* d_img_norm_out, float* d_anchors_f32_out);

int dodt_project_anchors_f32(dodt_ctx* ctx, const float* d_anchors, int n,
                             const int32_t* d_n, const float bev_extents[4],
                             const float p2[12], float im_w, float im_h,
                             float* d_bev_out, float* d_bev_norm_tf_out,
                             float* d_img_norm_tf_out);

int dodt_img_preprocess(dodt_ctx* ctx, const uint8_t* d_img_u8, int in_h, int in_w,
                        int out_h, int out_w, int out_c, const float mean_rgb[3],
                        float* d_out);

typedef struct dodt_extractor dodt_extractor;
#define DODT_EXTRACTOR_VGG_PYR 0
#define DODT_EXTRACTOR_VGG 1
#define DODT_EXTRACTOR_SHARED_GPU 0x100
#define DODT_EXTRACTOR_BF16 0x200
#define DODT_EXTRACTOR_SPLIT 0x400
#define DODT_CONV_MODE_DEFAULT 2
int dodt_conv_mode(void);
int dodt_extractor_create(dodt_ctx* ctx, int kind, int in_h, int in_w, int in_c,
                          int pad_top, int batch, dodt_extractor** out);
int dodt_extractor_destroy(dodt_extractor* ex);
int dodt_extractor_set_layer(dodt_extractor* ex, const char* name, const float* w,
                             int kh, int kw, int c_a, int c_b, const float* beta,
                             const float* mean, const float* var);
int dodt_extractor_input(dodt_extractor* ex, float** d_ptr, long long* frame_stride_floats);
int dodt_extractor_forward(dodt_extractor* ex, const float* d_in, float* d_feat_out,
                           float* d_bottleneck_out);
int dodt_extractor_forward_padded(dodt_extractor* ex, const float* d_x0, float* d_feat_out,
                                  float* d_bottleneck_out);
int dodt_extractor_set_input(dodt_extractor* ex, const float* d_x0);
int dodt_extractor_set_input_support(dodt_extractor* ex, const uint8_t* mask, int rows, int cols,
                                     long long* skipped_items);
int dodt_extractor_set_frame_tables(dodt_extractor* ex, int on, int* enabled);
int dodt_extractor_frame_items(dodt_extractor* ex, int* items, int n);
int dodt_extractor_frame_split(dodt_extractor* ex, int* computed, int* restored, int n);
long long dodt_extractor_store_bytes(const dodt_extractor* ex);
int dodt_frame_tables_host(const uint8_t* masks, int frames, int rows, int cols, int layer, int th, int tw,
                           const int* items, int n_items, const uint8_t* prev, int* run, int* n_run);
int dodt_frame_lists_host(const uint8_t* masks, int frames, int rows, int cols, int layer, int th, int tw,
                          const int* items, int n_items, const uint8_t* prev, int* run, int* n_run, int* restore,
                          int* n_restore);
int dodt_frame_restore_host(const int* item, int f, int th, int tw, int bn, int ch0, int rows, int cols, int channels,
                            int pad_top, float* dst, const float* src, float* dst2, const float* src2);
int dodt_extractor_output_shape(const dodt_extractor* ex, int* h, int* w, int* c);
int dodt_extractor_first_layers_folded(const dodt_extractor* ex);
int dodt_extractor_read_activation(dodt_extractor* ex, const char* name, float* dst,
                                   int* h, int* w, int* c);
double dodt_extractor_flops(const dodt_extractor* ex);
double dodt_extractor_mfma_flops(const dodt_extractor* ex);
double dodt_extractor_bytes(const dodt_extractor* ex);
typedef struct dodt_layer_info {
    char name[32];
    char kernel[48];
    int32_t launches;
    int32_t items;
    double flops_direct;
    double flops_executed;
    double bytes;
    float ms;
    int32_t reserved_;
} dodt_layer_info;
int dodt_extractor_layer_count(const dodt_extractor* ex);
int dodt_extractor_forward_timed(dodt_extractor* ex, const float* d_in, float* d_feat_out,
                                 float* d_bottleneck_out, dodt_layer_info* info, int n_info);

int dodt_crop_and_resize(dodt_ctx* ctx, const float* d_image, int H, int W, int C,
                         const float* d_boxes, int n, const int32_t* d_n, int crop_h,
                         int crop_w, float* d_out);
int dodt_crop_and_resize_strided(dodt_ctx* ctx, const float* d_image, int H, int W, int C,
                                 const float* d_boxes, int n, const int32_t* d_n, int crop_h,
                                 int crop_w, float* d_out, long long out_box_stride);
int dodt_crop_and_resize_indexed(dodt_ctx* ctx, const float* d_image, int H, int W, int C,
                                 const float* d_boxes, int n_boxes, const int32_t* d_box_idx, int n,
                                 const int32_t* d_n, int crop_h, int crop_w, float* d_out,
                                 long long out_box_stride);

int dodt_correlation(dodt_ctx* ctx, const float* d_a, const float* d_b, int H, int W, int C,
                     int max_displacement, int stride_2, int pad, float* d_out);
int dodt_correlation_tile_list(dodt_ctx* ctx, int OH, int OW, const float* d_boxes, int n_boxes,
                               const int32_t* d_box_idx, int n, const int32_t* d_n, int crop_h, int crop_w,
                               int32_t* d_tiles, int capacity, int32_t* d_n_tiles);
int dodt_correlation_tiles(dodt_ctx* ctx, const float* d_a, const float* d_b, int H, int W, int C,
                           int max_displacement, int stride_2, int pad, const int32_t* d_tiles, int capacity,
                           const int32_t* d_n_tiles, float* d_out);

int dodt_mean_fusion(dodt_ctx* ctx, const float* d_a, const float* d_b, int rows, const int32_t* d_n,
                     int row_floats, float* d_out);
typedef struct dodt_fc dodt_fc;
int dodt_fc_create(dodt_ctx* ctx, int K, int N, const float* w, const float* bias, int relu,
                   dodt_fc** out);
#define DODT_FC_RELU 1
#define DODT_FC_BF16 2
int dodt_fc_create_ex(dodt_ctx* ctx, int K, int N, const float* w, const float* bias, int flags,
                      dodt_fc** out);
int dodt_fc_destroy(dodt_fc* fc);
int dodt_fc_forward(dodt_fc* fc, dodt_ctx* ctx, const float* d_x, const float* d_x2, int ldx,
                    int M, const int32_t* d_m, float* d_y, int ldy);
int dodt_fc_forward_split(dodt_fc* fc, dodt_ctx* ctx, const float* d_x, int ldx, int M, const int32_t* d_m,
                          int parts, const int* widths, float* const* d_ys);
int dodt_fc_bf16_row_elems(const dodt_fc* fc);
int dodt_fc_forward_bf16(dodt_fc* fc, dodt_ctx* ctx, const void* d_x_bf16, int ldx, int M, const int32_t* d_m,
                         void* d_y, int ldy, int y_bf16);
int dodt_fc_forward_split_bf16(dodt_fc* fc, dodt_ctx* ctx, const void* d_x_bf16, int ldx, int M, const int32_t* d_m,
                               int parts, const int* widths, float* const* d_ys);
int dodt_rows_to_bf16(dodt_ctx* ctx, const float* d_a, const float* d_b, int rows, const int32_t* d_n,
                      int row_floats, int in_ld, void* d_out_bf16, int out_ld);
double dodt_fc_flops(const dodt_fc* fc, int M);

int dodt_nms(dodt_ctx* ctx, const float* d_boxes, const float* d_scores, int n,
             const int32_t* d_n, int max_out, float iou_threshold, int32_t* d_sel_out,
             int32_t* d_count_out);

int dodt_offset_to_anchor(dodt_ctx* ctx, const float* d_anchors, const float* d_offsets,
                          int n, const int32_t* d_n, float* d_out);
int dodt_softmax_fg(dodt_ctx* ctx, const float* d_logits2, int n, const int32_t* d_n,
                    float* d_scores_out);
int dodt_rpn_decode(dodt_ctx* ctx, const float* d_anchors, const float* d_offsets, const float* d_logits2, int n,
                    const int32_t* d_n, const float bev_extents[4], float* d_regressed_out,
                    float* d_bev_norm_tf_out, float* d_scores_out);
int dodt_gather_project(dodt_ctx* ctx, const float* d_src, const int32_t* d_idx, int n, const int32_t* d_n,
                        const float bev_extents[4], const float p2[12], float im_w, float im_h,
                        float* d_rows_out, float* d_bev_norm_tf_out, float* d_img_norm_tf_out);
int dodt_final_decode(dodt_ctx* ctx, const float* d_top_anchors, const float* d_offsets, const float* d_cls_logits2,
                      const float* d_angle_vectors, int n, const int32_t* d_n, const float plane[4],
                      const float bev_extents[4], float* d_boxes_3d_out, float* d_pred_anchors_out,
                      float* d_bev_tf_out, float* d_nms_scores_out, float* d_det_scores_out,
                      float* d_orientations_out);
int dodt_gather_rows(dodt_ctx* ctx, const float* d_src, int width, const int32_t* d_idx,
                     int n, const int32_t* d_n, float* d_out);
int dodt_max_fg_logit(dodt_ctx* ctx, const float* d_logits, int n_cls, int n,
                      const int32_t* d_n, float* d_scores_out);
int dodt_angle_vector_to_orientation(dodt_ctx* ctx, const float* d_angle_vectors, int n,
                                     const int32_t* d_n, float* d_orientations_out);
int dodt_pack_detections(dodt_ctx* ctx, const float* d_boxes_3d, const float* d_scores,
                         const float* d_orientations, const float* d_corr_offsets,
                         const int32_t* d_sel, const int32_t* d_count, int max_det,
                         float frame_mark, float* d_rec_out, int32_t* d_count_out);
int dodt_pack_detections_compact(dodt_ctx* ctx, const float* d_boxes_3d, const float* d_scores,
                                 const float* d_orientations, const float* d_det_offsets,
                                 const int32_t* d_sel, const int32_t* d_count, int max_det,
                                 float frame_mark, float* d_rec_out, int32_t* d_count_out);
int dodt_class_scores(dodt_ctx* ctx, const float* d_logits, int n_cls, int n, const int32_t* d_n,
                      float* d_scores_out, int32_t* d_types_out);
int dodt_final_decode_classes(dodt_ctx* ctx, const float* d_top_anchors, const float* d_offsets,
                              const float* d_cls_logits, int n_cls, const float* d_angle_vectors, int n,
                              const int32_t* d_n, const float plane[4], const float bev_extents[4],
                              float* d_boxes_3d_out, float* d_pred_anchors_out, float* d_bev_tf_out,
                              float* d_nms_scores_out, float* d_det_scores_out, int32_t* d_det_types_out,
                              float* d_orientations_out);
int dodt_pack_detections_classes(dodt_ctx* ctx, const float* d_boxes_3d, const float* d_scores, const int32_t* d_types,
                                 const float* d_orientations, const float* d_corr_offsets, const int32_t* d_sel,
                                 const int32_t* d_count, int max_det, float frame_mark, float* d_rec_out,
                                 int32_t* d_count_out);
int dodt_pack_detections_compact_classes(dodt_ctx* ctx, const float* d_boxes_3d, const float* d_scores,
                                         const int32_t* d_types, const float* d_orientations,
                                         const float* d_det_offsets, const int32_t* d_sel, const int32_t* d_count,
                                         int max_det, float frame_mark, float* d_rec_out, int32_t* d_count_out);
int dodt_box_4c_decode(dodt_ctx* ctx, const float* d_top_anchors, const float* d_offsets,
                       int n, const int32_t* d_n, const float plane[4],
                       const float bev_extents[4], float* d_boxes_3d_out,
                       float* d_pred_anchors_out, float* d_bev_tf_out);

int dodt_three_d_iou_matrix(dodt_ctx* ctx, const double* d_a, int na, const double* d_b, int nb,
                            double* d_iou_out);
#define DODT_CONFLICT_RAISE 0
#define DODT_CONFLICT_NEXT_BEST 1
int dodt_interpolate_pairs(dodt_ctx* ctx, const void* d_records, int records_f64, const int32_t* d_counts,
                           int n_pairs, int max_det, int n_frames, double threshold, int on_conflict,
                           const double* d_recover, const double* calib, int max_out, double* d_out,
                           int32_t* d_out_counts, int32_t* d_status);

int dodt_track_state_bytes(int log_capacity, size_t* bytes);
int dodt_track_reset(dodt_ctx* ctx, void* d_state, int log_capacity);
int dodt_track_flush(dodt_ctx* ctx, void* d_state, double high_threshold, int t_min);
int dodt_track_encode(dodt_ctx* ctx, const void* d_records, int records_f64, const int32_t* d_counts,
                      int n_pairs, int max_det, const double* p2, double image_w, double image_h,
                      double score_threshold, float* d_track_out, float* d_ious_out, int32_t* d_counts_out);
int dodt_track_pairs(dodt_ctx* ctx, void* d_state, const void* d_records, int records_f64,
                     const int32_t* d_counts, int n_pairs, int max_det, const double* p2, double image_w,
                     double image_h, double score_threshold, double high_threshold, double iou_threshold,
                     int t_min);
int dodt_track_encoded(dodt_ctx* ctx, void* d_state, const float* d_track, const float* d_ious,
                       const int32_t* d_counts, int n_pairs, int max_rows, double high_threshold,
                       double iou_threshold, int t_min);

typedef struct dodt_comm dodt_comm;
#define DODT_COMM_ID_BYTES 128
int dodt_comm_unique_id(uint8_t* id_out);
int dodt_comm_create(dodt_ctx* ctx, int rank, int world, const uint8_t* id, dodt_comm** out);
int dodt_comm_destroy(dodt_comm* comm);
int dodt_comm_attach(dodt_comm* comm, dodt_ctx* ctx);
int dodt_comm_rank(const dodt_comm* comm, int* rank, int* world);
int dodt_comm_set_late_peer(dodt_comm* comm, double microseconds);
int dodt_all_gather_records(dodt_comm* comm, dodt_ctx* producer, int slot, const float* d_records,
                            const int32_t* d_counts, int pairs, int frames, int max_det, int cols,
                            float* d_all_records, int32_t* d_all_counts);
int dodt_comm_join(dodt_comm* comm, int slot, dodt_ctx* consumer);
int dodt_comm_sync(dodt_comm* comm);
int dodt_comm_barrier(dodt_comm* comm);
int dodt_comm_max_f64(dodt_comm* comm, double* value);

#ifdef __cplusplus
}
#endif
#endif
```

Measured before the change: 419.5.

## Fuse RPN crops, FC head, and decode into one kernel

```diff
diff --git a/dodt_amd/_lib.py b/dodt_amd/_lib.py
--- a/dodt_amd/_lib.py
+++ b/dodt_amd/_lib.py
@@ -143,6 +143,8 @@
     'dodt_offset_to_anchor': (_i, [_vp, _pf, _pf, _i, _pi32, _pf]),
     'dodt_softmax_fg': (_i, [_vp, _pf, _i, _pi32, _pf]),
     'dodt_rpn_decode': (_i, [_vp, _pf, _pf, _pf, _i, _pi32, C.POINTER(_f), _pf, _pf, _pf]),
+    'dodt_rpn_stage': (_i, [_vp, _pf, _i, _i, _pf, _i, _i, _pf, _pf, _pf, _i, _vp, _vp, _vp, _vp, _i, _i,
+                            C.POINTER(_f), _pf, _pf, _pf, _pf, _pf, _pf, _pf]),
     'dodt_gather_project': (_i, [_vp, _pf, _pi32, _i, _pi32, C.POINTER(_f), C.POINTER(_f), _f, _f, _pf, _pf, _pf]),
     'dodt_final_decode': (_i, [_vp, _pf, _pf, _pf, _pf, _i, _pi32, C.POINTER(_f), C.POINTER(_f),
                                _pf, _pf, _pf, _pf, _pf, _pf]),
diff --git a/dodt_amd/core/models/anchor_predictor.py b/dodt_amd/core/models/anchor_predictor.py
--- a/dodt_amd/core/models/anchor_predictor.py
+++ b/dodt_amd/core/models/anchor_predictor.py
@@ -46,6 +46,17 @@
         self.cls8.forward(h7, n, d_objectness, ldx=2 * w, ctx=ctx)
         self.reg8.forward(h7.offset(4 * w, (1,)), n, d_offsets, ldx=2 * w, ctx=ctx)
 
+    def stage_eligible(self):
+        return (self.fc6.dtype == 'f32' and self.out8 is not None and self.fc6.K == 9 and self.width == 256 and
+                self.cls7.K == self.cls7.N == self.reg7.K == self.reg7.N == 256 and
+                (self.cls8.N, self.reg8.N) == (2, 6))
+
+    def forward_stage(self, ctx, d_bev_map, bev_hw, d_img_map, img_hw, d_bev_norm, d_img_norm, d_anchors, n,
+                      bev_extents, d_bev_roi, d_img_roi, d_objectness, d_offsets, d_regressed, d_prop_bev, d_scores):
+        ops.rpn_stage(ctx, d_bev_map, bev_hw, d_img_map, img_hw, d_bev_norm, d_img_norm, d_anchors, n, self.fc6,
+                      self.cls7, self.reg7, self.out8, self.cls8.N, self.reg8.N, bev_extents, d_bev_roi, d_img_roi,
+                      d_objectness, d_offsets, d_regressed, d_prop_bev, d_scores)
+
     def flops(self, n):
         return sum(l.flops(n) for l in self.layers)
 
diff --git a/dodt_amd/csrc/anchor_decode.h b/dodt_amd/csrc/anchor_decode.h
--- /dev/null
+++ b/dodt_amd/csrc/anchor_decode.h
@@ -0,0 +1,82 @@
+#pragma once
+
+namespace dodt {
+
+struct ProjParams32 {
+    float x_min, x_max, z_min, z_max;
+    float p[12];
+    float im_w, im_h;
+};
+
+__device__ __forceinline__ void bev_box32(float x, float z, float dx, float dz,
+                                          const ProjParams32& P, float& x1, float& z1,
+                                          float& x2, float& z2) {
+    const float hx = dx / 2.0f, hz = dz / 2.0f;
+    x1 = (x - hx) - P.x_min;
+    x2 = (x + hx) - P.x_min;
+    z1 = (P.z_max - (z + hz)) - P.z_min;
+    z2 = (P.z_max - (z - hz)) - P.z_min;
+}
+
+__device__ __forceinline__ void project_f32_elem(int i, float x, float y, float z, float dx, float dy, float dz,
+                                                 const ProjParams32& P, float* __restrict__ bev,
+                                                 float* __restrict__ bev_norm_tf, float* __restrict__ img_norm_tf) {
+    float x1, z1, x2, z2;
+    bev_box32(x, z, dx, dz, P, x1, z1, x2, z2);
+    if (bev) {
+        float* o = bev + (size_t)i * 4;
+        o[0] = x1; o[1] = z1; o[2] = x2; o[3] = z2;
+    }
+    if (bev_norm_tf) {
+        const float xr = P.x_max - P.x_min, zr = P.z_max - P.z_min;
+        float* o = bev_norm_tf + (size_t)i * 4;
+        o[0] = z1 / zr; o[1] = x1 / xr; o[2] = z2 / zr; o[3] = x2 / xr;
+    }
+    if (img_norm_tf) {
+        const float hx = dx / 2.0f, hz = dz / 2.0f;
+        const float xs[2] = {x + hx, x - hx};
+        const float ys[2] = {y, y - dy};
+        const float zs[2] = {z + hz, z - hz};
+        float umin = 3.0e38f, umax = -3.0e38f, vmin = 3.0e38f, vmax = -3.0e38f;
+#pragma unroll
+        for (int k = 0; k < 8; ++k) {
+            const float cx = xs[(k >> 1) & 1], cy = ys[k >> 2], cz = zs[((k + 1) >> 1) & 1];
+            const float un = ((P.p[0] * cx + P.p[1] * cy) + P.p[2] * cz) + P.p[3];
+            const float vn = ((P.p[4] * cx + P.p[5] * cy) + P.p[6] * cz) + P.p[7];
+            const float w = ((P.p[8] * cx + P.p[9] * cy) + P.p[10] * cz) + P.p[11];
+            const float u = un / w, v = vn / w;
+            umin = fminf(umin, u); umax = fmaxf(umax, u);
+            vmin = fminf(vmin, v); vmax = fmaxf(vmax, v);
+        }
+        float* o = img_norm_tf + (size_t)i * 4;
+        o[0] = vmin / P.im_h; o[1] = umin / P.im_w; o[2] = vmax / P.im_h; o[3] = umax / P.im_w;
+    }
+}
+
+__device__ __forceinline__ void offset_to_anchor_elem(const float* __restrict__ a, const float* __restrict__ t, float o[6]) {
+    o[0] = (t[0] * a[3]) + a[0];
+    o[1] = (t[1] * a[4]) + a[1];
+    o[2] = (t[2] * a[5]) + a[2];
+    o[3] = expf(logf(a[3]) + t[3]);
+    o[4] = expf(logf(a[4]) + t[4]);
+    o[5] = expf(logf(a[5]) + t[5]);
+}
+
+__device__ __forceinline__ float softmax_fg_elem(float l0, float l1) {
+    const float m = fmaxf(l0, l1);
+    const float e0 = expf(l0 - m), e1 = expf(l1 - m);
+    return e1 / (e0 + e1);
+}
+
+__device__ __forceinline__ void rpn_decode_elem(int i, const float* __restrict__ anchor, const float* __restrict__ off,
+                                                float l0, float l1, const ProjParams32& P, float* __restrict__ regressed,
+                                                float* __restrict__ bev_norm_tf, float* __restrict__ scores) {
+    float o[6];
+    offset_to_anchor_elem(anchor, off, o);
+#pragma unroll
+    for (int k = 0; k < 6; ++k) regressed[(size_t)i * 6 + k] = o[k];
+    project_f32_elem(i, o[0], o[1], o[2], o[3], o[4], o[5], P, nullptr, bev_norm_tf, nullptr);
+    scores[i] = softmax_fg_elem(l0, l1);
+}
+
+}
diff --git a/dodt_amd/csrc/anchors.hip b/dodt_amd/csrc/anchors.hip
--- a/dodt_amd/csrc/anchors.hip
+++ b/dodt_amd/csrc/anchors.hip
@@ -1,4 +1,5 @@
 #include "common.h"
+#include "anchor_decode.h"
 
 namespace {
 
@@ -125,56 +126,10 @@
     }
 }
 
-struct ProjParams32 {
-    float x_min, x_max, z_min, z_max;
-    float p[12];
-    float im_w, im_h;
-};
-
-__device__ __forceinline__ void bev_box32(float x, float z, float dx, float dz,
-                                          const ProjParams32& P, float& x1, float& z1,
-                                          float& x2, float& z2) {
-    const float hx = dx / 2.0f, hz = dz / 2.0f;
-    x1 = (x - hx) - P.x_min;
-    x2 = (x + hx) - P.x_min;
-    z1 = (P.z_max - (z + hz)) - P.z_min;
-    z2 = (P.z_max - (z - hz)) - P.z_min;
-}
-
-__device__ __forceinline__ void project_f32_elem(int i, float x, float y, float z, float dx, float dy, float dz,
-                                                 const ProjParams32& P, float* __restrict__ bev,
-                                                 float* __restrict__ bev_norm_tf, float* __restrict__ img_norm_tf) {
-    float x1, z1, x2, z2;
-    bev_box32(x, z, dx, dz, P, x1, z1, x2, z2);
-    if (bev) {
-        float* o = bev + (size_t)i * 4;
-        o[0] = x1; o[1] = z1; o[2] = x2; o[3] = z2;
-    }
-    if (bev_norm_tf) {
-        const float xr = P.x_max - P.x_min, zr = P.z_max - P.z_min;
-        float* o = bev_norm_tf + (size_t)i * 4;
-        o[0] = z1 / zr; o[1] = x1 / xr; o[2] = z2 / zr; o[3] = x2 / xr;
-    }
-    if (img_norm_tf) {
-        const float hx = dx / 2.0f, hz = dz / 2.0f;
-        const float xs[2] = {x + hx, x - hx};
-        const float ys[2] = {y, y - dy};
-        const float zs[2] = {z + hz, z - hz};
-        float umin = 3.0e38f, umax = -3.0e38f, vmin = 3.0e38f, vmax = -3.0e38f;
-#pragma unroll
-        for (int k = 0; k < 8; ++k) {
-            const float cx = xs[(k >> 1) & 1], cy = ys[k >> 2], cz = zs[((k + 1) >> 1) & 1];
-            const float un = ((P.p[0] * cx + P.p[1] * cy) + P.p[2] * cz) + P.p[3];
-            const float vn = ((P.p[4] * cx + P.p[5] * cy) + P.p[6] * cz) + P.p[7];
-            const float w = ((P.p[8] * cx + P.p[9] * cy) + P.p[10] * cz) + P.p[11];
-            const float u = un / w, v = vn / w;
-            umin = fminf(umin, u); umax = fmaxf(umax, u);
-            vmin = fminf(vmin, v); vmax = fmaxf(vmax, v);
-        }
-        float* o = img_norm_tf + (size_t)i * 4;
-        o[0] = vmin / P.im_h; o[1] = umin / P.im_w; o[2] = vmax / P.im_h; o[3] = umax / P.im_w;
-    }
-}
+using dodt::ProjParams32;
+using dodt::project_f32_elem;
+using dodt::offset_to_anchor_elem;
+using dodt::softmax_fg_elem;
 
 __global__ void __launch_bounds__(256)
 project_f32_kernel(const float* __restrict__ anchors, int n, const int* __restrict__ d_n,
@@ -187,15 +142,6 @@
     project_f32_elem(i, a[0], a[1], a[2], a[3], a[4], a[5], P, bev, bev_norm_tf, img_norm_tf);
 }
 
-__device__ __forceinline__ void offset_to_anchor_elem(const float* __restrict__ a, const float* __restrict__ t, float o[6]) {
-    o[0] = (t[0] * a[3]) + a[0];
-    o[1] = (t[1] * a[4]) + a[1];
-    o[2] = (t[2] * a[5]) + a[2];
-    o[3] = expf(logf(a[3]) + t[3]);
-    o[4] = expf(logf(a[4]) + t[4]);
-    o[5] = expf(logf(a[5]) + t[5]);
-}
-
 __global__ void __launch_bounds__(256)
 offset_to_anchor_kernel(const float* __restrict__ anchors, const float* __restrict__ off, int n,
                         const int* __restrict__ d_n, float* __restrict__ out) {
@@ -206,12 +152,6 @@
     offset_to_anchor_elem(anchors + (size_t)i * 6, off + (size_t)i * 6, o);
 #pragma unroll
     for (int k = 0; k < 6; ++k) out[(size_t)i * 6 + k] = o[k];
-}
-
-__device__ __forceinline__ float softmax_fg_elem(float l0, float l1) {
-    const float m = fmaxf(l0, l1);
-    const float e0 = expf(l0 - m), e1 = expf(l1 - m);
-    return e1 / (e0 + e1);
 }
 
 __global__ void __launch_bounds__(256)
@@ -230,12 +170,8 @@
     const int i = blockIdx.x * blockDim.x + threadIdx.x;
     const int lim = d_n ? min(*d_n, n) : n;
     if (i >= lim) return;
-    float o[6];
-    offset_to_anchor_elem(anchors + (size_t)i * 6, off + (size_t)i * 6, o);
-#pragma unroll
-    for (int k = 0; k < 6; ++k) regressed[(size_t)i * 6 + k] = o[k];
-    project_f32_elem(i, o[0], o[1], o[2], o[3], o[4], o[5], P, nullptr, bev_norm_tf, nullptr);
-    scores[i] = softmax_fg_elem(logits[2 * (size_t)i], logits[2 * (size_t)i + 1]);
+    dodt::rpn_decode_elem(i, anchors + (size_t)i * 6, off + (size_t)i * 6, logits[2 * (size_t)i], logits[2 * (size_t)i + 1], P,
+                          regressed, bev_norm_tf, scores);
 }
 
 __global__ void __launch_bounds__(256)
diff --git a/dodt_amd/csrc/crop.hip b/dodt_amd/csrc/crop.hip
--- a/dodt_amd/csrc/crop.hip
+++ b/dodt_amd/csrc/crop.hip
@@ -21,30 +21,19 @@
     const int src = box_idx ? box_idx[b] : b;
     const bool have = !box_idx || (src >= 0 && src < n_boxes);
     const float4 bx = have ? reinterpret_cast<const float4*>(boxes)[src] : make_float4(0.f, 0.f, 0.f, 0.f);
-    const float hm1 = (float)(H - 1), wm1 = (float)(W - 1);
-    const float in_y = dodt::crop_coord(bx.x, bx.z, H, ch, iy);
-    const float in_x = dodt::crop_coord(bx.y, bx.w, W, cw, ix);
+    const dodt::CropTaps s = dodt::crop_taps(bx.x, bx.y, bx.z, bx.w, H, W, ch, cw, iy, ix);
     float* o = out + (size_t)b * out_stride + (((size_t)iy * cw + ix) * C + (size_t)g * VEC);
-    const bool ok = have && (in_y >= 0.0f) && (in_y <= hm1) && (in_x >= 0.0f) && (in_x <= wm1);
-    if (!ok) {
+    if (!(have && s.ok)) {
 #pragma unroll
         for (int k = 0; k < VEC; ++k) o[k] = 0.0f;
         return;
     }
-    const int ty = (int)floorf(in_y), by = (int)ceilf(in_y);
-    const int lx_i = (int)floorf(in_x), rx_i = (int)ceilf(in_x);
-    const float ly = in_y - (float)ty, lx = in_x - (float)lx_i;
-    const float* ptl = img + ((size_t)ty * W + lx_i) * C + (size_t)g * VEC;
-    const float* ptr = img + ((size_t)ty * W + rx_i) * C + (size_t)g * VEC;
-    const float* pbl = img + ((size_t)by * W + lx_i) * C + (size_t)g * VEC;
-    const float* pbr = img + ((size_t)by * W + rx_i) * C + (size_t)g * VEC;
+    const float* ptl = img + ((size_t)s.ty * W + s.lx) * C + (size_t)g * VEC;
+    const float* ptr = img + ((size_t)s.ty * W + s.rx) * C + (size_t)g * VEC;
+    const float* pbl = img + ((size_t)s.by * W + s.lx) * C + (size_t)g * VEC;
+    const float* pbr = img + ((size_t)s.by * W + s.rx) * C + (size_t)g * VEC;
 #pragma unroll
-    for (int k = 0; k < VEC; ++k) {
-        const float tl = ptl[k], tr = ptr[k], bl = pbl[k], br = pbr[k];
-        const float top = tl + (tr - tl) * lx;
-        const float bot = bl + (br - bl) * lx;
-        o[k] = top + (bot - top) * ly;
-    }
+    for (int k = 0; k < VEC; ++k) o[k] = dodt::crop_blend(ptl[k], ptr[k], pbl[k], pbr[k], s.wx, s.wy);
 }
 
 int launch_crop(dodt_ctx* ctx, const float* d_image, int H, int W, int C, const float* d_boxes, int n,
diff --git a/dodt_amd/csrc/crop_coords.h b/dodt_amd/csrc/crop_coords.h
--- a/dodt_amd/csrc/crop_coords.h
+++ b/dodt_amd/csrc/crop_coords.h
@@ -8,4 +8,32 @@
     return (crop > 1) ? lo * m1 + (float)i * step : 0.5f * (lo + hi) * m1;
 }
 
+struct CropTaps {
+    bool ok;
+    int ty, by, lx, rx;
+    float wy, wx;
+};
+
+__device__ __forceinline__ CropTaps crop_taps(float y1, float x1, float y2, float x2, int H, int W, int crop_h,
+                                              int crop_w, int iy, int ix) {
+    const float hm1 = (float)(H - 1), wm1 = (float)(W - 1);
+    const float in_y = crop_coord(y1, y2, H, crop_h, iy);
+    const float in_x = crop_coord(x1, x2, W, crop_w, ix);
+    CropTaps t;
+    t.ok = (in_y >= 0.0f) && (in_y <= hm1) && (in_x >= 0.0f) && (in_x <= wm1);
+    t.ty = (int)floorf(in_y);
+    t.by = (int)ceilf(in_y);
+    t.lx = (int)floorf(in_x);
+    t.rx = (int)ceilf(in_x);
+    t.wy = in_y - (float)t.ty;
+    t.wx = in_x - (float)t.lx;
+    return t;
 }
+
+__device__ __forceinline__ float crop_blend(float tl, float tr, float bl, float br, float wx, float wy) {
+    const float top = tl + (tr - tl) * wx;
+    const float bot = bl + (br - bl) * wx;
+    return top + (bot - top) * wy;
+}
+
+}
diff --git a/dodt_amd/csrc/fc_layer.h b/dodt_amd/csrc/fc_layer.h
--- /dev/null
+++ b/dodt_amd/csrc/fc_layer.h
@@ -0,0 +1,17 @@
+#pragma once
+#include "common.h"
+
+struct dodt_fc {
+    dodt_ctx* ctx = nullptr;
+    int K = 0, Kp = 0, N = 0, Npad = 0, BN = 0, relu = 0;
+    bool bf16 = false;
+    float* d_w = nullptr;
+    float* d_b = nullptr;
+    float* d_w_plain = nullptr;
+    void* d_w_dma = nullptr;
+    int Kd = 0;
+    int dma_bk = 0;
+    bool smallk = false;
+    bool skinny = false;
+    bool dma = false;
+};
diff --git a/dodt_amd/csrc/gemm.hip b/dodt_amd/csrc/gemm.hip
--- a/dodt_amd/csrc/gemm.hip
+++ b/dodt_amd/csrc/gemm.hip
@@ -8,6 +8,7 @@
 #include <algorithm>
 
 #include "common.h"
+#include "fc_layer.h"
 #include "lds_dma.h"
 
 namespace {
@@ -787,20 +788,6 @@
     return DODT_OK;
 }
 
-struct dodt_fc {
-    dodt_ctx* ctx = nullptr;
-    int K = 0, Kp = 0, N = 0, Npad = 0, BN = 0, relu = 0;
-    bool bf16 = false;
-    float* d_w = nullptr;
-    float* d_b = nullptr;
-    float* d_w_plain = nullptr;
-    void* d_w_dma = nullptr;
-    int Kd = 0;
-    int dma_bk = 0;
-    bool smallk = false;
-    bool skinny = false;
-    bool dma = false;
-};
 
 namespace {
 
diff --git a/dodt_amd/csrc/rpn_stage.hip b/dodt_amd/csrc/rpn_stage.hip
--- /dev/null
+++ b/dodt_amd/csrc/rpn_stage.hip
@@ -0,0 +1,263 @@
+#include <mutex>
+
+#include "common.h"
+#include "anchor_decode.h"
+#include "crop_coords.h"
+#include "fc_layer.h"
+
+namespace {
+
+typedef float f32x16 __attribute__((ext_vector_type(16)));
+typedef float f32x4 __attribute__((ext_vector_type(4)));
+
+constexpr int kRows = 16;
+constexpr int kHidden = 256;
+constexpr int kLd = 2 * kHidden + 8;
+constexpr int kCropFloats = 2 * kRows * 9;
+constexpr int kOutLd = 32;
+constexpr int kOffOut = 320, kOffH = kOffOut + kRows * kOutLd;
+constexpr int kLdsFloats = kOffH + kRows * kLd;
+static_assert(kCropFloats <= kOffOut && 8 * 2 * 64 * 4 <= kRows * kLd, "LDS regions");
+
+struct RpnStageArgs {
+    const float* map[2];
+    int H[2], W[2];
+    const float* boxes[2];
+    float* roi[2];
+    const float* anchors;
+    int A;
+    const float* w6; const float* b6;
+    const float* w7[2]; const float* b7[2];
+    const float* w8; const float* b8;
+    int relu6, relu7[2], relu8;
+    int n_cls, n8;
+    dodt::ProjParams32 P;
+    float* logits; float* offsets; float* regressed; float* prop_bev; float* scores;
+};
+
+__global__ void __launch_bounds__(512, 8)
+rpn_stage_kernel(const RpnStageArgs a) {
+    extern __shared__ __attribute__((aligned(16))) float smem[];
+    float* s_crop = smem;
+    float* s_out = smem + kOffOut;
+    float* s_h = smem + kOffH;
+    const int tid = threadIdx.x, lane = tid & 63;
+    const int wave = __builtin_amdgcn_readfirstlane(tid >> 6);
+    const int m0 = blockIdx.x * kRows;
+
+    if (tid < kCropFloats) {
+        const int v = tid / (kRows * 9), r = tid - v * (kRows * 9);
+        const int i = r / 9, s = r - i * 9, m = m0 + i;
+        float val = 0.0f;
+        if (m < a.A) {
+            const float4 bx = reinterpret_cast<const float4*>(a.boxes[v])[m];
+            const int H = a.H[v], W = a.W[v];
+            const dodt::CropTaps t = dodt::crop_taps(bx.x, bx.y, bx.z, bx.w, H, W, 3, 3, s / 3, s % 3);
+            if (t.ok) {
+                const float* img = a.map[v];
+                val = dodt::crop_blend(img[(size_t)t.ty * W + t.lx], img[(size_t)t.ty * W + t.rx],
+                                       img[(size_t)t.by * W + t.lx], img[(size_t)t.by * W + t.rx], t.wx, t.wy);
+            }
+            a.roi[v][(size_t)m * 9 + s] = val;
+        }
+        s_crop[tid] = val;
+    }
+    __syncthreads();
+
+    {
+        const int c = (tid & 127) * 4, r0 = (tid >> 7) * 4;
+        const f32x4 b = *reinterpret_cast<const f32x4*>(a.b6 + c);
+        for (int rr = 0; rr < 4; ++rr) {
+            const int i = r0 + rr;
+            f32x4 acc = {0.f, 0.f, 0.f, 0.f};
+#pragma unroll
+            for (int k = 0; k < 9; ++k) {
+                float xv = s_crop[i * 9 + k];
+                xv = (xv + s_crop[kRows * 9 + i * 9 + k]) / 2.0f;
+                acc += *reinterpret_cast<const f32x4*>(a.w6 + k * (2 * kHidden) + c) * xv;
+            }
+            acc += b;
+            if (a.relu6) {
+#pragma unroll
+                for (int e = 0; e < 4; ++e) acc[e] = fmaxf(acc[e], 0.0f);
+            }
+            *reinterpret_cast<f32x4*>(s_h + i * kLd + c) = acc;
+        }
+    }
+    __syncthreads();
+
+    {
+        const int br = wave >> 2, n0 = (wave & 3) * 64;
+        const int li = lane & 31, lh = lane >> 5;
+        const auto wrsrc = __builtin_amdgcn_make_buffer_rsrc(const_cast<float*>(a.w7[br]), 0,
+                                                             kHidden * kHidden * (int)sizeof(float), 0x00020000);
+        const int wq = ((n0 / 128) * (kHidden / 8) * 2 * 128 + (n0 % 128)) * 16;
+        const int wl = (lh * 128 + li) * 16;
+        const float* xr = s_h + (li & 15) * kLd + br * kHidden + 4 * lh;
+        constexpr int QC = 2, NC = kHidden / 8 / QC;
+        float keep[2][8];
+#pragma unroll
+        for (int nt = 0; nt < 2; ++nt) {
+            const int wn = wq + nt * 32 * 16;
+            f32x16 acc;
+#pragma unroll
+            for (int r = 0; r < 16; ++r) acc[r] = 0.0f;
+            f32x4 wf[3][QC];
+            auto load_chunk = [&](int c) {
+#pragma unroll
+                for (int qq = 0; qq < QC; ++qq)
+                    wf[c % 3][qq] = __builtin_bit_cast(
+                        f32x4, __builtin_amdgcn_raw_buffer_load_b128(wrsrc, wl, wn + (c * QC + qq) * 4096, 0));
+            };
+            load_chunk(0);
+            load_chunk(1);
+#pragma unroll
+            for (int c = 0; c < NC; ++c) {
+                if (c + 2 < NC) load_chunk(c + 2);
+                __builtin_amdgcn_sched_barrier(0);
+#pragma unroll
+                for (int qq = 0; qq < QC; ++qq) {
+                    const f32x4 xf = *reinterpret_cast<const f32x4*>(xr + (c * QC + qq) * 8);
+#pragma unroll
+                    for (int s = 0; s < 4; ++s)
+                        acc = __builtin_amdgcn_mfma_f32_32x32x2f32(xf[s], wf[c % 3][qq][s], acc, 0, 0, 0);
+                }
+            }
+#pragma unroll
+            for (int r = 0; r < 8; ++r) keep[nt][r] = acc[r];
+        }
+        __syncthreads();
+#pragma unroll
+        for (int nt = 0; nt < 2; ++nt) {
+            const int n = n0 + nt * 32 + li;
+            const float b = a.b7[br][n];
+#pragma unroll
+            for (int r = 0; r < 8; ++r) {
+                float v = keep[nt][r] + b;
+                if (a.relu7[br]) v = fmaxf(v, 0.0f);
+                s_h[(4 * lh + (r & 3) + 8 * (r >> 2)) * kLd + br * kHidden + n] = v;
+            }
+        }
+    }
+    __syncthreads();
+    __builtin_amdgcn_sched_barrier(0);
+
+    f32x4* s_part = reinterpret_cast<f32x4*>(s_h);
+    const int i = lane & 15, g = lane >> 4;
+    {
+        const float* xr = s_h + i * kLd + 4 * g;
+        const f32x4* w4 = reinterpret_cast<const f32x4*>(a.w8) + g * 32 + i;
+        f32x4 acc0 = {0.f, 0.f, 0.f, 0.f}, acc1 = {0.f, 0.f, 0.f, 0.f};
+        f32x4 xv[4], wa[4], wb[4];
+#pragma unroll
+        for (int u = 0; u < 4; ++u) {
+            const int j = wave + 8 * u;
+            xv[u] = *reinterpret_cast<const f32x4*>(xr + 16 * j);
+            wa[u] = w4[(size_t)j * 128];
+            wb[u] = w4[(size_t)j * 128 + 16];
+        }
+        __syncthreads();
+#pragma unroll
+        for (int u = 0; u < 4; ++u)
+#pragma unroll
+            for (int s = 0; s < 4; ++s) {
+                acc0 = __builtin_amdgcn_mfma_f32_16x16x4f32(xv[u][s], wa[u][s], acc0, 0, 0, 0);
+                acc1 = __builtin_amdgcn_mfma_f32_16x16x4f32(xv[u][s], wb[u][s], acc1, 0, 0, 0);
+            }
+        s_part[(wave * 2 + 0) * 64 + lane] = acc0;
+        s_part[(wave * 2 + 1) * 64 + lane] = acc1;
+    }
+    __syncthreads();
+    if (tid < 128) {
+        const int nb = tid >> 6;
+        f32x4 sum = s_part[nb * 64 + lane];
+#pragma unroll
+        for (int w = 1; w < 8; ++w) sum += s_part[(w * 2 + nb) * 64 + lane];
+        const int n = nb * 16 + i;
+        if (n < a.n8) {
+            const float b = a.b8[n];
+            float* y = n < a.n_cls ? a.logits : a.offsets;
+            const int ld = n < a.n_cls ? a.n_cls : a.n8 - a.n_cls;
+            const int nn = n < a.n_cls ? n : n - a.n_cls;
+#pragma unroll
+            for (int r = 0; r < 4; ++r) {
+                float v = sum[r] + b;
+                if (a.relu8) v = fmaxf(v, 0.0f);
+                s_out[(4 * g + r) * kOutLd + n] = v;
+                const int m = m0 + 4 * g + r;
+                if (m < a.A) y[(size_t)m * ld + nn] = v;
+            }
+        }
+    }
+    __syncthreads();
+
+    if (tid < kRows && m0 + tid < a.A) {
+        const int m = m0 + tid;
+        const float* o = s_out + tid * kOutLd;
+        float off[6];
+#pragma unroll
+        for (int k = 0; k < 6; ++k) off[k] = o[2 + k];
+        dodt::rpn_decode_elem(m, a.anchors + (size_t)m * 6, off, o[0], o[1], a.P, a.regressed, a.prop_bev, a.scores);
+    }
+}
+
+}
+
+extern "C" int dodt_rpn_stage(dodt_ctx* ctx, const float* d_bev_map, int bev_h, int bev_w, const float* d_img_map,
+                              int img_h, int img_w, const float* d_bev_norm, const float* d_img_norm,
+                              const float* d_anchors, int n, const dodt_fc* fc6, const dodt_fc* cls7,
+                              const dodt_fc* reg7, const dodt_fc* out8, int n_cls, int n_reg,
+                              const float bev_extents[4], float* d_bev_roi_out, float* d_img_roi_out,
+                              float* d_logits_out, float* d_offsets_out, float* d_regressed_out,
+                              float* d_bev_norm_tf_out, float* d_scores_out) {
+    DODT_REQUIRE(ctx && d_bev_map && d_img_map && bev_extents && fc6 && cls7 && reg7, "dodt_rpn_stage: NULL argument");
+    DODT_REQUIRE(bev_h > 0 && bev_w > 0 && img_h > 0 && img_w > 0 && n >= 0, "dodt_rpn_stage: bad sizes");
+    DODT_REQUIRE(n == 0 || (d_bev_norm && d_img_norm && d_anchors && d_bev_roi_out && d_img_roi_out && d_logits_out &&
+                            d_offsets_out && d_regressed_out && d_bev_norm_tf_out && d_scores_out),
+                 "dodt_rpn_stage: NULL argument");
+    const char* why = nullptr;
+    if (!out8) why = "the output layers are not one split layer";
+    else if (fc6->bf16 || cls7->bf16 || reg7->bf16 || out8->bf16) why = "bf16 layers";
+    else if (fc6->K != 9 || !fc6->d_w_plain) why = "fc6 is not a 3x3x1 layer";
+    else if (fc6->N != 2 * kHidden || cls7->K != kHidden || cls7->N != kHidden || reg7->K != kHidden ||
+             reg7->N != kHidden || cls7->BN != 128 || reg7->BN != 128 || cls7->Kp != kHidden || reg7->Kp != kHidden ||
+             out8->K != 2 * kHidden)
+        why = "a hidden width other than 256 per branch";
+    else if (n_cls != 2 || n_reg != 6 || out8->N != n_cls + n_reg || out8->Npad != kOutLd)
+        why = "output columns other than 2 | 6";
+    else if (((size_t)d_bev_norm | (size_t)d_img_norm) % 16 != 0 ||
+             ((size_t)d_bev_map | (size_t)d_img_map | (size_t)d_anchors | (size_t)d_bev_roi_out | (size_t)d_img_roi_out |
+              (size_t)d_logits_out | (size_t)d_offsets_out | (size_t)d_regressed_out | (size_t)d_bev_norm_tf_out |
+              (size_t)d_scores_out) % 4 != 0)
+        why = "a misaligned pointer (boxes: 16 bytes, everything else: 4)";
+    if (why) {
+        dodt::set_error("dodt_rpn_stage: %s", why);
+        return DODT_ERR_UNSUPPORTED;
+    }
+    if (n == 0) return DODT_OK;
+    RpnStageArgs a = {};
+    a.map[0] = d_bev_map; a.H[0] = bev_h; a.W[0] = bev_w; a.boxes[0] = d_bev_norm; a.roi[0] = d_bev_roi_out;
+    a.map[1] = d_img_map; a.H[1] = img_h; a.W[1] = img_w; a.boxes[1] = d_img_norm; a.roi[1] = d_img_roi_out;
+    a.anchors = d_anchors;
+    a.A = n;
+    a.w6 = fc6->d_w_plain; a.b6 = fc6->d_b; a.relu6 = fc6->relu;
+    a.w7[0] = cls7->d_w; a.b7[0] = cls7->d_b; a.relu7[0] = cls7->relu;
+    a.w7[1] = reg7->d_w; a.b7[1] = reg7->d_b; a.relu7[1] = reg7->relu;
+    a.w8 = out8->d_w; a.b8 = out8->d_b; a.relu8 = out8->relu;
+    a.n_cls = n_cls; a.n8 = out8->N;
+    a.P.x_min = bev_extents[0]; a.P.x_max = bev_extents[1];
+    a.P.z_min = bev_extents[2]; a.P.z_max = bev_extents[3];
+    a.logits = d_logits_out; a.offsets = d_offsets_out; a.regressed = d_regressed_out;
+    a.prop_bev = d_bev_norm_tf_out; a.scores = d_scores_out;
+    constexpr size_t lds = (size_t)kLdsFloats * sizeof(float);
+    static std::once_flag once;
+    static hipError_t allowed = hipSuccess;
+    std::call_once(once, [] {
+        allowed = hipFuncSetAttribute(reinterpret_cast<const void*>(&rpn_stage_kernel),
+                                      hipFuncAttributeMaxDynamicSharedMemorySize, (int)lds);
+    });
+    DODT_HIP_CHECK(allowed);
+    hipLaunchKernelGGL(rpn_stage_kernel, dim3(dodt::ceil_div(n, kRows)), dim3(512), lds, ctx->stream, a);
+    DODT_LAUNCH_CHECK();
+    return DODT_OK;
+}
diff --git a/dodt_amd/ops.py b/dodt_amd/ops.py
--- a/dodt_amd/ops.py
+++ b/dodt_amd/ops.py
@@ -191,6 +191,16 @@
         _p(d_regressed), _p(d_bev_norm_tf), _p(d_scores)), 'dodt_rpn_decode')
 
 
+def rpn_stage(ctx, d_bev_map, bev_hw, d_img_map, img_hw, d_bev_norm, d_img_norm, d_anchors, n, fc6, cls7, reg7, out8,
+              n_cls, n_reg, bev_extents, d_bev_roi, d_img_roi, d_logits, d_offsets, d_regressed, d_bev_norm_tf, d_scores):
+    h = [None if l is None else l.handle for l in (fc6, cls7, reg7, out8)]
+    _lib.check(ctx.lib.dodt_rpn_stage(
+        ctx.handle, _p(d_bev_map), int(bev_hw[0]), int(bev_hw[1]), _p(d_img_map), int(img_hw[0]), int(img_hw[1]),
+        _p(d_bev_norm), _p(d_img_norm), _p(d_anchors), int(n), h[0], h[1], h[2], h[3], int(n_cls), int(n_reg),
+        _arr(C.c_float, bev_extents), _p(d_bev_roi), _p(d_img_roi), _p(d_logits), _p(d_offsets), _p(d_regressed),
+        _p(d_bev_norm_tf), _p(d_scores)), 'dodt_rpn_stage')
+
+
 def gather_project(ctx, d_src, d_idx, n, d_n, bev_extents, p2, im_wh, d_rows, d_bev_norm_tf, d_img_norm_tf):
     _lib.check(ctx.lib.dodt_gather_project(
         ctx.handle, _p(d_src), _p(d_idx), int(n), _p(d_n), _arr(C.c_float, bev_extents), _arr(C.c_float, p2),
diff --git a/dodt_amd/pipeline.py b/dodt_amd/pipeline.py
--- a/dodt_amd/pipeline.py
+++ b/dodt_amd/pipeline.py
@@ -76,7 +76,7 @@
                  image_wh=_config.KITTI_IMAGE_WH, n_points_max=120000, rpn_nms_size=1024,
                  pairs_per_step=1, side_streams=None, head_params=None, conv_dtype='f32',
                  head_dtype='f32', reuse_streams_of=None, temporal=None, tracker=None,
-                 bev_input_skip=True, bev_frame_tables=True, t_branch_rows=None, sequence=False):
+                 bev_input_skip=True, bev_frame_tables=True, t_branch_rows=None, sequence=False, fused_rpn=None):
         self.sequence = bool(sequence)
         if self.sequence and (int(cfg.get('frames_per_sample', 2)) != 2 or int(pairs_per_step) != 1):
             raise ValueError('sequence: needs frames_per_sample == 2 and pairs_per_step == 1')
@@ -154,6 +154,7 @@
         f32, i32 = np.float32, np.int32
         N, P = self.n_all, self.P
         self.rpn_head = self.avod_head = self.corr_head = self.head_scratch = None
+        self.fused_rpn = False
         rep = cfg.get('box_representation', 'box_4ca')
         if rep not in ('box_4c', 'box_4ca'):
             raise NotImplementedError('Regression not implemented for %s' % rep)
@@ -166,6 +167,8 @@
             if self.fps == 2:
                 self.corr_head = EarlyFusionFcLayers(ctx, head_params['corr'],
                                                      outputs=('off_out',), dtype=head_dtype)
+            self.fused_rpn = (fused_rpn is None or bool(fused_rpn)) and head_dtype == 'f32' and \
+                self.rpn_head.stage_eligible()
             self.head_scratch = [dict(rpn=self.rpn_head.make_scratch(N), fc=self.avod_head.make_scratch(P),
                                       corr_map=ctx.empty((self.bev_fh, self.bev_fw, CORR_CH), f32)
                                       if self.fps == 2 else None) for _ in self.sides]
@@ -770,6 +773,13 @@
         c, b, h, A, v = self.sides[f % len(self.sides)], t.fr[f], t.heads[f], t.counts[f], t.feat[f]
         bev_hw, img_hw, FC = (self.bev_fh, self.bev_fw), (self.img_fh, self.img_fw), self.feat_c
         self._mark(c, t.step, 'tail%d_start' % f)
+        if self.fused_rpn and self.sched.fused_tail and not self.sched.no_rpn and h is b:
+            self.rpn_head.forward_stage(c, v['bev_bneck'], bev_hw, v['img_bneck'], img_hw, b['bev_norm'], b['img_norm'],
+                                        b['anchors'], A, self.bev_extents_flat, b['rpn_bev_roi'], b['rpn_img_roi'],
+                                        b['rpn_logits'], b['rpn_offsets'], b['regressed'], b['prop_bev'], b['scores'])
+            self._mark(c, t.step, 'tail%d_crops' % f)
+            self._mark(c, t.step, 'tail%d_rpn' % f)
+            return self._proposals_nms1(t, f)
         ops.crop_and_resize(c, v['bev_bneck'], bev_hw + (1,), b['bev_norm'], A, None, (3, 3), b['rpn_bev_roi'])
         ops.crop_and_resize(c, v['img_bneck'], img_hw + (1,), b['img_norm'], A, None, (3, 3), b['rpn_img_roi'])
         self._mark(c, t.step, 'tail%d_crops' % f)
@@ -785,6 +795,11 @@
             ops.project_anchors_f32(c, b['regressed'], A, None, self.bev_extents_flat, self.p2,
                                     self.image_wh, d_bev_norm_tf=b['prop_bev'])
             ops.softmax_fg(c, h['rpn_logits'], A, None, b['scores'])
+        self._proposals_nms1(t, f)
+
+    def _proposals_nms1(self, t, f):
+        c, b, A, v = self.sides[f % len(self.sides)], t.fr[f], t.counts[f], t.feat[f]
+        bev_hw, img_hw, FC = (self.bev_fh, self.bev_fw), (self.img_fh, self.img_fw), self.feat_c
         ops.nms(c, b['prop_bev'], b['scores'], A, None, self.P, self.cfg['rpn_nms_iou_thresh'], b['top_idx'], b['top_count'])
         if self.sched.fused_tail:
             ops.gather_project(c, b['regressed'], b['top_idx'], self.P, b['top_count'], self.bev_extents_flat,
diff --git a/include/dodt_hip.h b/include/dodt_hip.h
--- a/include/dodt_hip.h
+++ b/include/dodt_hip.h
@@ -197,6 +197,12 @@
 int dodt_rpn_decode(dodt_ctx* ctx, const float* d_anchors, const float* d_offsets, const float* d_logits2, int n,
                     const int32_t* d_n, const float bev_extents[4], float* d_regressed_out,
                     float* d_bev_norm_tf_out, float* d_scores_out);
+int dodt_rpn_stage(dodt_ctx* ctx, const float* d_bev_map, int bev_h, int bev_w, const float* d_img_map, int img_h,
+                   int img_w, const float* d_bev_norm, const float* d_img_norm, const float* d_anchors, int n,
+                   const dodt_fc* fc6, const dodt_fc* cls7, const dodt_fc* reg7, const dodt_fc* out8, int n_cls,
+                   int n_reg, const float bev_extents[4], float* d_bev_roi_out, float* d_img_roi_out,
+                   float* d_logits_out, float* d_offsets_out, float* d_regressed_out, float* d_bev_norm_tf_out,
+                   float* d_scores_out);
 int dodt_gather_project(dodt_ctx* ctx, const float* d_src, const int32_t* d_idx, int n, const int32_t* d_n,
                         const float bev_extents[4], const float p2[12], float im_w, float im_h,
                         float* d_rows_out, float* d_bev_norm_tf_out, float* d_img_norm_tf_out);
```

Result: no change. 423.3 (median of 6 runs) (+0.9%).
